# musevlt/muse-psfr

Measured on AMD Instinct MI355X. Metric: PSFs/sec (row x lambda) on 512^2 grid, 35 lambda, higher is better.
Workload: dtype f64 PSD->structure function, per-lambda OTF f32 -> split-fp16 MFMA (fp32 accumulate), f64 fit

## Files before the change

### muse_psfr_amd/csrc/dpp_groups.h

```cpp
#pragma once
#include "fft_lds.h"

namespace mpsfr {
namespace {

template <int L0>
__device__ __forceinline__ void cmac_group1(cx<double>& a0, double xr0, double xi0, const cx<double>& w) {
    asm("v_fmac_f64_dpp %0, %2, %4 row_newbcast:%6 row_mask:0xf bank_mask:0xf\n\t"
        "v_fmac_f64_dpp %1, %2, %5 row_newbcast:%6 row_mask:0xf bank_mask:0xf\n\t"
        "v_fmac_f64_dpp %0, -%3, %5 row_newbcast:%6 row_mask:0xf bank_mask:0xf\n\t"
        "v_fmac_f64_dpp %1, %3, %4 row_newbcast:%6 row_mask:0xf bank_mask:0xf"
        : "+v"(a0.x), "+v"(a0.y)
        : "v"(xr0), "v"(xi0), "v"(w.x), "v"(w.y), "n"(L0));
}

template <int L0>
__device__ __forceinline__ void rmac_group1(cx<double>& a0, double xr0, const cx<double>& w) {
    asm("v_fmac_f64_dpp %0, %2, %3 row_newbcast:%5 row_mask:0xf bank_mask:0xf\n\t"
        "v_fmac_f64_dpp %1, %2, %4 row_newbcast:%5 row_mask:0xf bank_mask:0xf"
        : "+v"(a0.x), "+v"(a0.y)
        : "v"(xr0), "v"(w.x), "v"(w.y), "n"(L0));
}

template <int L0, int L1>
__device__ __forceinline__ void cmac_group2(cx<double>& a0, cx<double>& a1, double xr0, double xi0, double xr1, double xi1, const cx<double>& w) {
    asm("v_fmac_f64_dpp %0, %4, %8 row_newbcast:%10 row_mask:0xf bank_mask:0xf\n\t"
        "v_fmac_f64_dpp %2, %6, %8 row_newbcast:%11 row_mask:0xf bank_mask:0xf\n\t"
        "v_fmac_f64_dpp %1, %4, %9 row_newbcast:%10 row_mask:0xf bank_mask:0xf\n\t"
        "v_fmac_f64_dpp %3, %6, %9 row_newbcast:%11 row_mask:0xf bank_mask:0xf\n\t"
        "v_fmac_f64_dpp %0, -%5, %9 row_newbcast:%10 row_mask:0xf bank_mask:0xf\n\t"
        "v_fmac_f64_dpp %2, -%7, %9 row_newbcast:%11 row_mask:0xf bank_mask:0xf\n\t"
        "v_fmac_f64_dpp %1, %5, %8 row_newbcast:%10 row_mask:0xf bank_mask:0xf\n\t"
        "v_fmac_f64_dpp %3, %7, %8 row_newbcast:%11 row_mask:0xf bank_mask:0xf"
        : "+v"(a0.x), "+v"(a0.y), "+v"(a1.x), "+v"(a1.y)
        : "v"(xr0), "v"(xi0), "v"(xr1), "v"(xi1), "v"(w.x), "v"(w.y), "n"(L0), "n"(L1));
}

template <int L0, int L1>
__device__ __forceinline__ void rmac_group2(cx<double>& a0, cx<double>& a1, double xr0, double xr1, const cx<double>& w) {
    asm("v_fmac_f64_dpp %0, %4, %6 row_newbcast:%8 row_mask:0xf bank_mask:0xf\n\t"
        "v_fmac_f64_dpp %2, %5, %6 row_newbcast:%9 row_mask:0xf bank_mask:0xf\n\t"
        "v_fmac_f64_dpp %1, %4, %7 row_newbcast:%8 row_mask:0xf bank_mask:0xf\n\t"
        "v_fmac_f64_dpp %3, %5, %7 row_newbcast:%9 row_mask:0xf bank_mask:0xf"
        : "+v"(a0.x), "+v"(a0.y), "+v"(a1.x), "+v"(a1.y)
        : "v"(xr0), "v"(xr1), "v"(w.x), "v"(w.y), "n"(L0), "n"(L1));
}

template <int L0, int L1, int L2, int L3>
__device__ __forceinline__ void cmac_group4(cx<double>& a0, cx<double>& a1, cx<double>& a2, cx<double>& a3, double xr0, double xi0, double xr1, double xi1, double xr2, double xi2, double xr3, double xi3, const cx<double>& w) {
    asm("v_fmac_f64_dpp %0, %8, %16 row_newbcast:%18 row_mask:0xf bank_mask:0xf\n\t"
        "v_fmac_f64_dpp %2, %10, %16 row_newbcast:%19 row_mask:0xf bank_mask:0xf\n\t"
        "v_fmac_f64_dpp %4, %12, %16 row_newbcast:%20 row_mask:0xf bank_mask:0xf\n\t"
        "v_fmac_f64_dpp %6, %14, %16 row_newbcast:%21 row_mask:0xf bank_mask:0xf\n\t"
        "v_fmac_f64_dpp %1, %8, %17 row_newbcast:%18 row_mask:0xf bank_mask:0xf\n\t"
        "v_fmac_f64_dpp %3, %10, %17 row_newbcast:%19 row_mask:0xf bank_mask:0xf\n\t"
        "v_fmac_f64_dpp %5, %12, %17 row_newbcast:%20 row_mask:0xf bank_mask:0xf\n\t"
        "v_fmac_f64_dpp %7, %14, %17 row_newbcast:%21 row_mask:0xf bank_mask:0xf\n\t"
        "v_fmac_f64_dpp %0, -%9, %17 row_newbcast:%18 row_mask:0xf bank_mask:0xf\n\t"
        "v_fmac_f64_dpp %2, -%11, %17 row_newbcast:%19 row_mask:0xf bank_mask:0xf\n\t"
        "v_fmac_f64_dpp %4, -%13, %17 row_newbcast:%20 row_mask:0xf bank_mask:0xf\n\t"
        "v_fmac_f64_dpp %6, -%15, %17 row_newbcast:%21 row_mask:0xf bank_mask:0xf\n\t"
        "v_fmac_f64_dpp %1, %9, %16 row_newbcast:%18 row_mask:0xf bank_mask:0xf\n\t"
        "v_fmac_f64_dpp %3, %11, %16 row_newbcast:%19 row_mask:0xf bank_mask:0xf\n\t"
        "v_fmac_f64_dpp %5, %13, %16 row_newbcast:%20 row_mask:0xf bank_mask:0xf\n\t"
        "v_fmac_f64_dpp %7, %15, %16 row_newbcast:%21 row_mask:0xf bank_mask:0xf"
        : "+v"(a0.x), "+v"(a0.y), "+v"(a1.x), "+v"(a1.y), "+v"(a2.x), "+v"(a2.y), "+v"(a3.x), "+v"(a3.y)
        : "v"(xr0), "v"(xi0), "v"(xr1), "v"(xi1), "v"(xr2), "v"(xi2), "v"(xr3), "v"(xi3), "v"(w.x), "v"(w.y), "n"(L0), "n"(L1), "n"(L2), "n"(L3));
}

template <int L0, int L1, int L2, int L3>
__device__ __forceinline__ void rmac_group4(cx<double>& a0, cx<double>& a1, cx<double>& a2, cx<double>& a3, double xr0, double xr1, double xr2, double xr3, const cx<double>& w) {
    asm("v_fmac_f64_dpp %0, %8, %12 row_newbcast:%14 row_mask:0xf bank_mask:0xf\n\t"
        "v_fmac_f64_dpp %2, %9, %12 row_newbcast:%15 row_mask:0xf bank_mask:0xf\n\t"
        "v_fmac_f64_dpp %4, %10, %12 row_newbcast:%16 row_mask:0xf bank_mask:0xf\n\t"
        "v_fmac_f64_dpp %6, %11, %12 row_newbcast:%17 row_mask:0xf bank_mask:0xf\n\t"
        "v_fmac_f64_dpp %1, %8, %13 row_newbcast:%14 row_mask:0xf bank_mask:0xf\n\t"
        "v_fmac_f64_dpp %3, %9, %13 row_newbcast:%15 row_mask:0xf bank_mask:0xf\n\t"
        "v_fmac_f64_dpp %5, %10, %13 row_newbcast:%16 row_mask:0xf bank_mask:0xf\n\t"
        "v_fmac_f64_dpp %7, %11, %13 row_newbcast:%17 row_mask:0xf bank_mask:0xf"
        : "+v"(a0.x), "+v"(a0.y), "+v"(a1.x), "+v"(a1.y), "+v"(a2.x), "+v"(a2.y), "+v"(a3.x), "+v"(a3.y)
        : "v"(xr0), "v"(xr1), "v"(xr2), "v"(xr3), "v"(w.x), "v"(w.y), "n"(L0), "n"(L1), "n"(L2), "n"(L3));
}

template <int L0, int L1, int L2, int L3, int L4>
__device__ __forceinline__ void cmac_group5(cx<double>& a0, cx<double>& a1, cx<double>& a2, cx<double>& a3, cx<double>& a4, double xr0, double xi0, double xr1, double xi1, double xr2, double xi2, double xr3, double xi3, double xr4, double xi4, const cx<double>& w) {
    asm("v_fmac_f64_dpp %0, %10, %20 row_newbcast:%22 row_mask:0xf bank_mask:0xf\n\t"
        "v_fmac_f64_dpp %2, %12, %20 row_newbcast:%23 row_mask:0xf bank_mask:0xf\n\t"
        "v_fmac_f64_dpp %4, %14, %20 row_newbcast:%24 row_mask:0xf bank_mask:0xf\n\t"
        "v_fmac_f64_dpp %6, %16, %20 row_newbcast:%25 row_mask:0xf bank_mask:0xf\n\t"
        "v_fmac_f64_dpp %8, %18, %20 row_newbcast:%26 row_mask:0xf bank_mask:0xf\n\t"
        "v_fmac_f64_dpp %1, %10, %21 row_newbcast:%22 row_mask:0xf bank_mask:0xf\n\t"
        "v_fmac_f64_dpp %3, %12, %21 row_newbcast:%23 row_mask:0xf bank_mask:0xf\n\t"
        "v_fmac_f64_dpp %5, %14, %21 row_newbcast:%24 row_mask:0xf bank_mask:0xf\n\t"
        "v_fmac_f64_dpp %7, %16, %21 row_newbcast:%25 row_mask:0xf bank_mask:0xf\n\t"
        "v_fmac_f64_dpp %9, %18, %21 row_newbcast:%26 row_mask:0xf bank_mask:0xf\n\t"
        "v_fmac_f64_dpp %0, -%11, %21 row_newbcast:%22 row_mask:0xf bank_mask:0xf\n\t"
        "v_fmac_f64_dpp %2, -%13, %21 row_newbcast:%23 row_mask:0xf bank_mask:0xf\n\t"
        "v_fmac_f64_dpp %4, -%15, %21 row_newbcast:%24 row_mask:0xf bank_mask:0xf\n\t"
        "v_fmac_f64_dpp %6, -%17, %21 row_newbcast:%25 row_mask:0xf bank_mask:0xf\n\t"
        "v_fmac_f64_dpp %8, -%19, %21 row_newbcast:%26 row_mask:0xf bank_mask:0xf\n\t"
        "v_fmac_f64_dpp %1, %11, %20 row_newbcast:%22 row_mask:0xf bank_mask:0xf\n\t"
        "v_fmac_f64_dpp %3, %13, %20 row_newbcast:%23 row_mask:0xf bank_mask:0xf\n\t"
        "v_fmac_f64_dpp %5, %15, %20 row_newbcast:%24 row_mask:0xf bank_mask:0xf\n\t"
        "v_fmac_f64_dpp %7, %17, %20 row_newbcast:%25 row_mask:0xf bank_mask:0xf\n\t"
        "v_fmac_f64_dpp %9, %19, %20 row_newbcast:%26 row_mask:0xf bank_mask:0xf"
        : "+v"(a0.x), "+v"(a0.y), "+v"(a1.x), "+v"(a1.y), "+v"(a2.x), "+v"(a2.y), "+v"(a3.x), "+v"(a3.y), "+v"(a4.x), "+v"(a4.y)
        : "v"(xr0), "v"(xi0), "v"(xr1), "v"(xi1), "v"(xr2), "v"(xi2), "v"(xr3), "v"(xi3), "v"(xr4), "v"(xi4), "v"(w.x), "v"(w.y), "n"(L0), "n"(L1), "n"(L2), "n"(L3), "n"(L4));
}

template <int L0, int L1, int L2, int L3, int L4>
__device__ __forceinline__ void rmac_group5(cx<double>& a0, cx<double>& a1, cx<double>& a2, cx<double>& a3, cx<double>& a4, double xr0, double xr1, double xr2, double xr3, double xr4, const cx<double>& w) {
    asm("v_fmac_f64_dpp %0, %10, %15 row_newbcast:%17 row_mask:0xf bank_mask:0xf\n\t"
        "v_fmac_f64_dpp %2, %11, %15 row_newbcast:%18 row_mask:0xf bank_mask:0xf\n\t"
        "v_fmac_f64_dpp %4, %12, %15 row_newbcast:%19 row_mask:0xf bank_mask:0xf\n\t"
        "v_fmac_f64_dpp %6, %13, %15 row_newbcast:%20 row_mask:0xf bank_mask:0xf\n\t"
        "v_fmac_f64_dpp %8, %14, %15 row_newbcast:%21 row_mask:0xf bank_mask:0xf\n\t"
        "v_fmac_f64_dpp %1, %10, %16 row_newbcast:%17 row_mask:0xf bank_mask:0xf\n\t"
        "v_fmac_f64_dpp %3, %11, %16 row_newbcast:%18 row_mask:0xf bank_mask:0xf\n\t"
        "v_fmac_f64_dpp %5, %12, %16 row_newbcast:%19 row_mask:0xf bank_mask:0xf\n\t"
        "v_fmac_f64_dpp %7, %13, %16 row_newbcast:%20 row_mask:0xf bank_mask:0xf\n\t"
        "v_fmac_f64_dpp %9, %14, %16 row_newbcast:%21 row_mask:0xf bank_mask:0xf"
        : "+v"(a0.x), "+v"(a0.y), "+v"(a1.x), "+v"(a1.y), "+v"(a2.x), "+v"(a2.y), "+v"(a3.x), "+v"(a3.y), "+v"(a4.x), "+v"(a4.y)
        : "v"(xr0), "v"(xr1), "v"(xr2), "v"(xr3), "v"(xr4), "v"(w.x), "v"(w.y), "n"(L0), "n"(L1), "n"(L2), "n"(L3), "n"(L4));
}

}
}
```

### muse_psfr_amd/csrc/kernels.h

```cpp
#pragma once
#include <hip/hip_runtime.h>
#include <stdint.h>

namespace mpsfr {

constexpr int NS = 40;
constexpr int NSH = NS / 2 + 1;
constexpr int KS = 41;
constexpr int NAO = 80;
constexpr int NFIT = 16;
constexpr int NFIT_ELL = 24;
constexpr int NFIT_PSF = 16;
constexpr int METRIC_MAX = 16;
constexpr int METRIC_HEAD = 8;
constexpr int KHAT = 33 * 64;
constexpr int MAXLGS = 4;

struct TaskPar {
    double r0m53;
    double inv_l0sq;
    double cn2_0;
    double cn2_1;
    int geom;
    int basis;
};

struct LamPar {
    double c;
    int npixc;
    int pad;
};

struct AoGeom {
    double h[2];
    double wind[2][2];
    int nlgs[2];
    double poslgs[2][2][MAXLGS];
    int ndir;
    double dir[2][25];
};

constexpr int MAXLAYER = 8;
struct AoLayers {
    int n;
    int ntab;
    double h[MAXLAYER];
    double wind[2][MAXLAYER];
};
inline int ao_ntab(int nlayer) { return nlayer < 2 ? 2 : nlayer; }
struct LayerMix {
    const double* w = nullptr;
    int ntab = 2;
};

constexpr int kMfLists = 64;
constexpr int kMfSchedInts = kMfLists + 1;

enum KernelId {
    K_AO_TABLES = 0,
    K_TEL_OTF,
    K_PSD_ROWFFT,
    K_COLFFT_DPHI,
    K_GTABLE,
    K_MOFFAT_KERNELS,
    K_OTF_ROWFFT,
    K_COLPASS,
    K_CONV,
    K_FIT,
    K_STAMP_SUM,
    K_VKEEP,
    K_OTF_MFMA,
    K_MF_PREP,
    K_PATCH,
    K_DPHI_SERIES,
    K_COUNT
};

void launch_ao_tables(hipStream_t s, const AoGeom& g, const uint8_t* d_mask_rec,
                      const uint8_t* d_mask_res, double* d_tab);
void launch_ao_tables_profile(hipStream_t s, const AoGeom& g, const AoLayers& ly, const uint8_t* d_mask_rec,
                              const uint8_t* d_mask_res, double* d_tab);
void launch_tel_otf(hipStream_t s, int N, const uint64_t* d_rows, int words, double pupsum,
                    void* d_tel, bool f64out);
int psd_rowfft_groups(int N);
void launch_psd_rowfft(hipStream_t s, int N, int ntd, int ndir, const TaskPar* d_tp,
                       const double* d_aotab, double cfit, void* d_C, const void* d_tw64,
                       double* d_dcpart, bool f64, const LayerMix& mix = LayerMix());
void launch_colfft_dphi(hipStream_t s, int N, int ntd, const void* d_C, const double* d_dcpart,
                        double scale2, void* d_D0t, bool f64out, const void* d_tw64,
                        int* d_zero = nullptr);
void launch_dmin(hipStream_t s, int N, int ntd, const void* d_D0t, float* d_dline, float* d_dblk,
                 bool f64 = false);
void launch_psd_image(hipStream_t s, int N, int ndir, const TaskPar& p, const double* d_aotab, double cfit,
                      double unit, double* d_psd, const LayerMix& mix = LayerMix());
void launch_dphi_from_psd(hipStream_t s, int N, int ndir, const double* d_psd, void* d_Cm, double scale,
                          void* d_D0t, bool f64out, const void* d_tw64);
bool p2p_supported(int M);
void launch_p2p_otf(hipStream_t s, int M, int P, int nz, const double* d_pup, const double* d_phase,
                    const double* d_lbda_m, double scale, void* d_T1, void* d_Q, double* d_otft, const void* d_twm);
void launch_p2p_psf(hipStream_t s, int M, int N, int nz, const double* d_D0t, const double* d_otft, size_t otf_stride,
                    const double* d_cl, void* d_G, double* d_psf, const void* d_twm);
size_t series_twiddle_bytes(int N);
void launch_series_twiddles(hipStream_t s, int N, const void* d_tw64, void* d_twk);
int series_terms(bool f64);
double series_eps0();
inline double series_eps_max() { return 1.0 / 49.0; }
void launch_series_coef(hipStream_t s, int N, const double* d_planes, void* d_coef, bool f64);
struct SeriesQueue {
    int* queue = nullptr;
    const int* perm = nullptr;
    const float* tlmax = nullptr;
    float c2max = 0.f, thr_elem = -3.0e38f, thr_mass = -3.0e38f;
};
struct PatchExtras {
    const void* blob_src = nullptr;
    void* blob_dst = nullptr;
    size_t blob_bytes = 0;
    const TaskPar* tp_host = nullptr;
    unsigned long long* flag = nullptr;
    unsigned long long seq = 0;
    int* queue_zero = nullptr;
    int khat_n = 0;
    const double* khat_gam = nullptr;
    const double* khat_alp = nullptr;
    void* khat_out = nullptr;
    bool khat_f64 = false;
};
void launch_patch(hipStream_t s, int N, int ntd, int ndir, const TaskPar* d_tp, const double* d_aotab,
                  double cfit, const void* d_twk, double* d_P, void* d_T, double* d_sp, bool f64,
                  const PatchExtras& x = PatchExtras(), const LayerMix& mix = LayerMix());
void launch_dphi_series(hipStream_t s, int N, int ntd, int ndir, const TaskPar* d_tp, const void* d_T,
                        const double* d_sp, const void* d_coef, const void* d_twk, double scale2,
                        void* d_D0t, float* d_dlin, bool f64out, int* d_zero, int ncu,
                        const unsigned* d_support = nullptr, const SeriesQueue& qx = SeriesQueue());
void launch_series_support(hipStream_t s, int N, const void* d_tel, bool f64, unsigned* d_support);
void launch_dmin16(hipStream_t s, int N, int ntd, const float* d_dlin, float* d_dline, float* d_dblk);
void launch_tel_linemax(hipStream_t s, int N, const void* d_tel, float* d_tlmax, bool f64 = false);
void launch_vkeep(hipStream_t s, int N, int ntask, int ndir, int nl, const LamPar* d_lp,
                  const float* d_dline, const float* d_dblk, const float* d_tlmax, float thr_sum,
                  int* d_vkeep, int fixed, float* d_dminb);
void launch_task_order(hipStream_t s, int ntask, int nl, const int* d_vkeep, int* d_order);
size_t mf_etab_bytes(int N, int nl);
size_t mf_gtab_bytes(int N, int nl);
size_t mf_tl2_bytes(int N);
size_t mf_tlb_bytes(int N);
size_t mf_dminb_bytes(int N, int ntask);
int mf_block_count(int N);
void launch_mf_tables(hipStream_t s, int N, int nl, const LamPar* d_lp, const void* d_tw64,
                      void* d_E, void* d_G);
void launch_mf_tel(hipStream_t s, int N, const void* d_tel, float* d_tl2, float* d_tlb);
void launch_peak_floor(hipStream_t s, int N, int ntask, int ndir, const void* d_D0t, const float* d_tl2, float c2min,
                       float tier_half, float floor_nominal, float* d_thrf);
void launch_otf_mfma(hipStream_t s, int N, int ntask, int ndir, int nl, const void* d_D0t,
                     const float* d_tl2, const LamPar* d_lp, const void* d_E, const void* d_G,
                     const int* d_vkeep, const float* d_dminb, const float* d_tlb, float thr,
                     void* d_pre, const int* d_order = nullptr, void* d_clk = nullptr, const float* d_thrf = nullptr);
size_t mf2_own_bytes(int N, int ntask, int nl);
size_t mf2_uni_bytes(int N, int ntask, int nl);
size_t mf2_sched_bytes(int N, int ntask, int nl, int permax);
size_t mf2_part_bytes(int N, int ntask, int nl);
void mf2_groups(int nl, int permax, int* per, int* ngr);
void launch_mf_prep(hipStream_t s, int N, int ntask, int nl, int permax, const LamPar* d_lp,
                    const float* d_dminb, const float* d_tlb, float thr, float thr_floor, float thr_mid,
                    float tier_half, const void* d_D0t, const float* d_tl2, void* d_own,
                    void* d_uni, void* d_sched, const float* d_dlin = nullptr);
void launch_otf_mfma2(hipStream_t s, int N, int ntask, int nl, int permax, int ncu, const void* d_D0t,
                      const float* d_tl2, const LamPar* d_lp, const void* d_E, const void* d_G,
                      const void* d_own, const void* d_uni, void* d_sched, void* d_part, void* d_pre,
                      void* d_clk = nullptr, hipEvent_t ev_start = nullptr, hipEvent_t ev_stop = nullptr,
                      bool finish = true);
struct MfFinishArgs {
    const int* gsw = nullptr;
    const void* part = nullptr;
    int per = 1, ngr = 1, nsw = 1;
};
MfFinishArgs mf2_finish_args(int N, int ntask, int nl, int permax, void* d_sched, const void* d_part);
void launch_mf_finish(hipStream_t s, int N, int ntask, int nl, int permax, void* d_sched, const void* d_part, void* d_pre);
void launch_gtable(hipStream_t s, int N, int nl, const LamPar* d_lp, const void* d_tw64,
                   int* d_samp_p, void* d_samp_a, void* d_G, bool f64);
void launch_moffat_kernels(hipStream_t s, int nker, const double* d_gamma, const double* d_alpha,
                           void* d_out, bool f64);
void launch_otf_rowfft(hipStream_t s, int N, int ntask, int ndir, int nl, const void* d_D0t,
                       const void* d_tel, const LamPar* d_lp, const int* d_samp_p,
                       const void* d_samp_a, const void* d_xtab, void* d_Tq, const void* d_tw64,
                       bool f64, bool fast_exp, const int* d_vkeep);
bool otf_uses_r16(int N, bool f64, int nl, int ndir);
size_t xtab_bytes(int nl);
void launch_xtab(hipStream_t s, int N, int nl, const int* d_samp_p, const void* d_samp_a,
                 const void* d_tw64, void* d_xtab);
void launch_colpass(hipStream_t s, int N, int ntask, int nl, const void* d_Tq, const void* d_G,
                    void* d_pre, bool f64, const int* d_vkeep);
void launch_conv(hipStream_t s, int ntask, int nl, const void* d_pre, const void* d_ktt,
                 const void* d_kmuse, double* d_fin, bool f64, int tdiv = 1);
void launch_khat(hipStream_t s, int nker, const double* d_gamma, const double* d_alpha,
                 void* d_khat, bool f64 = false);
void launch_conv_fft(hipStream_t s, int ntask, int nl, const void* d_pre, const void* d_khat_tt,
                     const void* d_khat_muse, void* d_fin, bool fin_f32, bool f64 = false,
                     const MfFinishArgs& finish = MfFinishArgs(), int tdiv = 1);
void launch_fit(hipStream_t s, int nstamp, const void* d_stamps, bool stamps_f32, double* d_fit,
                bool f64, int sum_ntask = 0, int sum_nl = 0, double* d_sum = nullptr, int sum_accumulate = 0);
void launch_stamp_sum(hipStream_t s, int ntask, int nl, const void* d_fin, bool fin_f32, double* d_sum,
                      int accumulate);
void launch_fit_ell(hipStream_t s, int nstamp, const double* d_stamps, double* d_fit, bool f64);
void launch_fit_obs(hipStream_t s, int nstamp, const double* d_stamps, const double* d_var, int flags, double* d_fit,
                    bool f64);
void launch_fit_psf(hipStream_t s, int nstamp, const double* d_stamps, const double* d_var, int npsf,
                    const double* d_psf, const int32_t* d_index, const double* d_shift, int flags, double* d_fit,
                    bool f64);
void launch_stamp_metrics(hipStream_t s, int nstamp, const double* d_stamps, const double* d_centers, int nrad,
                          const double* radii, int nbox, const double* boxes, int nfrac, const double* fractions,
                          double* d_out);
constexpr int MAX_BANDS = 16;
int band_stride(int nband);
void launch_band_reduce(hipStream_t s, int ntb, int nl, int nband, const void* d_fin, bool fin_f32,
                        const double* d_w, double* d_out);
void launch_param_copy(hipStream_t s, void* d_dst, const void* h_src_pinned, size_t bytes,
                       unsigned long long* h_flag_pinned = nullptr, unsigned long long seq = 0);

}
```

### muse_psfr_amd/csrc/mpsfr_api.cpp

```cpp
#include "../../include/mpsfr.h"

#include <hip/hip_runtime.h>

#include <algorithm>
#include <chrono>
#include <cmath>
#include <cstdarg>
#include <cstdio>
#include <cstring>
#include <string>
#include <thread>
#include <vector>

#include "coeff_l0_table.h"
#include "kernels.h"

using namespace mpsfr;

namespace {

thread_local std::string g_err;

constexpr float kMfFloorLog2 = -29.01f;

// ... 784 lines not shown
static_assert(MAX_BANDS == MPSFR_MAX_BANDS, "K_BAND_REDUCE keeps MPSFR_MAX_BANDS accumulators");

int mpsfr_reconstruct_band(mpsfr_ctx* c, int ntask, const double* seeing, const double* gl, const double* l0,
                           const uint8_t* three_lgs, const double h[2], double wind_speed, int npsflin, int npos,
                           const double* pos_arcsec, int nl, const double* lbda_nm, int nband, const double* weights,
                           const uint8_t* mask_rec, const uint8_t* mask_res, double* band_out, double* band_sum_out,
                           double* band_fit_out, int on_device) {
    if (!c) return fail(MPSFR_E_INVALID, "ctx is NULL");
    if (nband < 1 || nband > MPSFR_MAX_BANDS) return fail(MPSFR_E_INVALID, "nband=%d out of range 1..%d", nband, MPSFR_MAX_BANDS);
    if (nl < 1 || nl > 4096) return fail(MPSFR_E_INVALID, "nl=%d out of range", nl);
    if (!weights) return fail(MPSFR_E_INVALID, "weights is NULL");
    std::vector<double> w((size_t)nband * nl);
    for (int b = 0; b < nband; ++b) {
        const double* r = weights + (size_t)b * nl;
        double sum = 0.0;
        for (int l = 0; l < nl; ++l) {
            if (!std::isfinite(r[l]) || r[l] < 0.0) return fail(MPSFR_E_INVALID, "band %d: weight %d must be finite and >= 0", b, l);
            sum += r[l];
        }
        if (!(sum > 0.0) || !std::isfinite(sum)) return fail(MPSFR_E_INVALID, "band %d: the weights sum to %g", b, sum);
        for (int l = 0; l < nl; ++l) w[(size_t)b * nl + l] = r[l] / sum;
    }
    StageIO io;
    io.nband = nband;
    io.bw = w.data();
    if (npos < 0 || npos > 25) return fail(MPSFR_E_INVALID, "npos=%d out of range 0..25", npos);
    if (npos > 0) {
        if (npsflin != 0) return fail(MPSFR_E_INVALID, "a field call (npos >= 1) takes npsflin = 0");
        if (!pos_arcsec) return fail(MPSFR_E_INVALID, "pos_arcsec is NULL");
        for (int k = 0; k < 2 * npos; ++k)
            if (!std::isfinite(pos_arcsec[k]) || std::fabs(pos_arcsec[k]) > 60.0)
                return fail(MPSFR_E_INVALID, "position %d: need finite |x|, |y| <= 60 arcsec", k / 2);
        io.npos = npos;
        io.pos = pos_arcsec;
        npsflin = 1;
    } else if (npsflin < 1 || npsflin > 5) {
        return fail(MPSFR_E_INVALID, "npsflin=%d out of range 1..5", npsflin);
    }
    return guarded_call(c, ntask, seeing, gl, l0, three_lgs, h, wind_speed, npsflin, nl, lbda_nm, mask_rec, mask_res,
                        band_out, band_sum_out, band_fit_out, on_device, io);
}

static_assert(MAXLAYER == MPSFR_MAX_LAYERS, "AoLayers holds MPSFR_MAX_LAYERS layers");

static int profile_layers(int ntask, int nlayer, const double* h, const double* wind_speed, const double* wind_dir,
                          const double* cn2, AoLayers& ly, std::vector<double>& w) {
    if (nlayer < 1 || nlayer > MPSFR_MAX_LAYERS) return fail(MPSFR_E_INVALID, "nlayer=%d out of range 1..%d", nlayer, MPSFR_MAX_LAYERS);
    if (!h || !wind_speed || !wind_dir || !cn2) return fail(MPSFR_E_INVALID, "NULL profile array");
    memset(&ly, 0, sizeof ly);
    ly.n = nlayer;
    ly.ntab = ao_ntab(nlayer);
    for (int l = 0; l < nlayer; ++l) {
        if (!std::isfinite(h[l]) || !std::isfinite(wind_speed[l]) || !std::isfinite(wind_dir[l]))
            return fail(MPSFR_E_INVALID, "layer %d: non-finite altitude or wind", l);
        if (h[l] < 0.0 || h[l] > 50000.0) return fail(MPSFR_E_INVALID, "layer %d: h=%g outside [0, 50000] m", l, h[l]);
        if (wind_speed[l] < 0.0 || wind_speed[l] > 100.0)
            return fail(MPSFR_E_INVALID, "layer %d: wind speed %g outside [0, 100] m/s", l, wind_speed[l]);
        ly.h[l] = h[l];
        ly.wind[0][l] = wind_speed[l] * std::cos(wind_dir[l]);
        ly.wind[1][l] = wind_speed[l] * std::sin(wind_dir[l]);
    }
    for (int t = 0; t < ntask; ++t) {
        double sum = 0.0;
        for (int l = 0; l < nlayer; ++l) {
            const double w = cn2[(size_t)t * nlayer + l];
            if (!std::isfinite(w) || w < 0.0) return fail(MPSFR_E_INVALID, "row %d: weight %d must be finite and >= 0", t, l);
            sum += w;
        }
        if (!(sum > 0.0) || !std::isfinite(sum)) return fail(MPSFR_E_INVALID, "row %d: the weights sum to %g", t, sum);
    }
    int keep[MAXLAYER], nk = 0;
    for (int l = 0; l < nlayer; ++l) {
        bool used = false;
        for (int t = 0; t < ntask && !used; ++t) used = cn2[(size_t)t * nlayer + l] != 0.0;
        if (used) keep[nk++] = l;
    }
    for (int k = 0; k < nk; ++k) {
        ly.h[k] = ly.h[keep[k]];
        ly.wind[0][k] = ly.wind[0][keep[k]];
        ly.wind[1][k] = ly.wind[1][keep[k]];
    }
    for (int k = nk; k < MAXLAYER; ++k) ly.h[k] = ly.wind[0][k] = ly.wind[1][k] = 0.0;
    ly.n = nk;
    ly.ntab = ao_ntab(nk);
    w.resize((size_t)ntask * nk);
    for (int t = 0; t < ntask; ++t)
        for (int k = 0; k < nk; ++k) w[(size_t)t * nk + k] = cn2[(size_t)t * nlayer + keep[k]];
    return MPSFR_OK;
}

int mpsfr_reconstruct_profile(mpsfr_ctx* c, int ntask, const double* seeing, const double* gl,
                              const double* l0, const uint8_t* three_lgs,
                              int nlayer, const double* h, const double* wind_speed, const double* wind_dir,
                              const double* cn2, int npsflin, int npos, const double* pos_arcsec,
                              int nl, const double* lbda_nm, const uint8_t* mask_rec, const uint8_t* mask_res,
                              double* psf_out, double* psf_sum_out, double* fit_out, int on_device) {
    if (!c) return fail(MPSFR_E_INVALID, "ctx is NULL");
    if (ntask < 1) return fail(MPSFR_E_INVALID, "ntask < 1");
    AoLayers ly;
    std::vector<double> w;
    int rc = profile_layers(ntask, nlayer, h, wind_speed, wind_dir, cn2, ly, w);
    if (rc) return rc;
    StageIO io;
    io.layers = &ly;
    io.cn2 = w.data();
    if (npos < 0 || npos > 25) return fail(MPSFR_E_INVALID, "npos=%d out of range 0..25", npos);
    if (npos > 0) {
        if (npsflin != 0) return fail(MPSFR_E_INVALID, "a field call (npos >= 1) takes npsflin = 0");
        if (!pos_arcsec) return fail(MPSFR_E_INVALID, "pos_arcsec is NULL");
        for (int k = 0; k < 2 * npos; ++k)
            if (!std::isfinite(pos_arcsec[k]) || std::fabs(pos_arcsec[k]) > 60.0)
                return fail(MPSFR_E_INVALID, "position %d: need finite |x|, |y| <= 60 arcsec", k / 2);
        io.npos = npos;
        io.pos = pos_arcsec;
        npsflin = 1;
    } else if (npsflin < 1 || npsflin > 5) {
        return fail(MPSFR_E_INVALID, "npsflin=%d out of range 1..5", npsflin);
    }
    const double h2[2] = {0.0, 0.0};
    return guarded_call(c, ntask, seeing, gl, l0, three_lgs, h2, 0.0, npsflin, nl, lbda_nm, mask_rec, mask_res,
                        psf_out, psf_sum_out, fit_out, on_device, io);
}

int mpsfr_simul_psd_profile(mpsfr_ctx* c, double seeing, double l0, int three_lgs,
                            int nlayer, const double* h, const double* wind_speed, const double* wind_dir,
                            const double* cn2, int npsflin, int npos, const double* pos_arcsec,
                            const uint8_t* mask_rec, const uint8_t* mask_res, double* psd_out) {
    if (!c || !psd_out) return fail(MPSFR_E_INVALID, "NULL argument");
    AoLayers ly;
    std::vector<double> w;
    int rc = profile_layers(1, nlayer, h, wind_speed, wind_dir, cn2, ly, w);
    if (rc) return rc;
    StageIO io;
    io.layers = &ly;
    io.cn2 = w.data();
    io.psd_out = psd_out;
    if (npos < 0 || npos > 25) return fail(MPSFR_E_INVALID, "npos=%d out of range 0..25", npos);
    if (npos > 0) {
        if (npsflin != 0) return fail(MPSFR_E_INVALID, "positions (npos >= 1) take npsflin = 0");
        if (!pos_arcsec) return fail(MPSFR_E_INVALID, "pos_arcsec is NULL");
        for (int k = 0; k < 2 * npos; ++k)
            if (!std::isfinite(pos_arcsec[k]) || std::fabs(pos_arcsec[k]) > 60.0)
                return fail(MPSFR_E_INVALID, "position %d: need finite |x|, |y| <= 60 arcsec", k / 2);
        io.npos = npos;
        io.pos = pos_arcsec;
        npsflin = 1;
    } else if (npsflin < 1 || npsflin > 5) {
        return fail(MPSFR_E_INVALID, "npsflin=%d out of range 1..5", npsflin);
    }
    const uint8_t t3 = three_lgs ? 1 : 0;
    const double lb = 700.0;
    const double h2[2] = {0.0, 0.0};
    const double gl = 0.5;
    return guarded_call(c, 1, &seeing, &gl, &l0, &t3, h2, 0.0, npsflin, 1, &lb, mask_rec, mask_res,
                        nullptr, nullptr, nullptr, 0, io);
}

static int reconstruct_impl(mpsfr_ctx* c, int ntask, const double* seeing, const double* gl,
                            const double* l0, const uint8_t* three_lgs, const double h[2],
                            double wind_speed, int npsflin, int nl, const double* lbda_nm,
                            const uint8_t* mask_rec, const uint8_t* mask_res, double* psf_out,
                            double* psf_sum_out, double* fit_out, int on_device, const StageIO& io) {
    const auto t_enter = std::chrono::steady_clock::now();
    const bool staged = io.psd_out || io.psd_in || io.pre_in || io.stop_pre;
    if (staged && on_device != 0) return fail(MPSFR_E_INVALID, "stage-level calls take host buffers");
    if (ntask < 1 || !seeing || !gl || !l0 || !h || !lbda_nm)
        return fail(MPSFR_E_INVALID, "ntask < 1 or NULL input array");
    if (nl < 1 || nl > 4096) return fail(MPSFR_E_INVALID, "nl=%d out of range", nl);
    const bool field = io.npos > 0;
    if (field && ((staged && !io.psd_out) || !io.pos)) return fail(MPSFR_E_INVALID, "field call without positions");
    if (!field && (npsflin < 1 || npsflin > 5)) return fail(MPSFR_E_INVALID, "npsflin=%d out of range 1..5", npsflin);
    if ((mask_rec == nullptr) != (mask_res == nullptr))
        return fail(MPSFR_E_INVALID, "mask_rec and mask_res must both be given or both be NULL");
    const int N = c->N, H1 = N / 2 + 1, ndir = field ? io.npos : npsflin * npsflin;
    const int gpp = field ? ndir : 1, ndb = field ? 1 : ndir;
    const bool band = io.nband > 0;
    if (band && (staged || !io.bw || io.nband > MAX_BANDS)) return fail(MPSFR_E_INVALID, "bad band request");
    const int nout = band ? io.nband : nl;
    HIPCHK(hipSetDevice(c->device));
    int rc;

    std::vector<LamPar> lp(nl);
    std::vector<double> gam, alp;
    for (int l = 0; l < nl; ++l) {
        if (!(lbda_nm[l] > 0.0)) return fail(MPSFR_E_INVALID, "lbda[%d] must be > 0", l);
        const double k = 2.0 * M_PI / lbda_nm[l];
        lp[l].c = -0.5 * k * k;
        lp[l].npixc = npix_crop(lbda_nm[l], c->dimpsf, c->pixscale);
        lp[l].pad = 0;
        if (!io.pre_in && !io.psd_out && (lp[l].npixc > N || lp[l].npixc < NS))
            return fail(MPSFR_E_GRID,
                        "lbda=%.3f nm needs a %d-pixel crop, outside [%d, dim=%d] "
                        "(psfrec.py:663-683)", lbda_nm[l], lp[l].npixc, NS, N);
    }
    const AoLayers* ly = io.layers;
    const int ntab = ly ? ly->ntab : 2;
    std::vector<double> wts;
    int low = 0;
    if (ly) {
        if (!io.cn2) return fail(MPSFR_E_INVALID, "profile call without weights");
        wts.assign((size_t)ntask * ntab, 0.0);
        for (int l = 1; l < ly->n; ++l)
            if (ly->h[l] < ly->h[low]) low = l;
        for (int t = 0; t < ntask; ++t) {
            const double* r = io.cn2 + (size_t)t * ly->n;
            double sum = 0.0;
            for (int l = 0; l < ly->n; ++l) sum += r[l];
            for (int l = 0; l < ly->n; ++l) wts[(size_t)t * ntab + l] = r[l] / sum;
        }
    }
    std::vector<TaskPar> tp(ntask);
    gam.resize((size_t)ntask + nl);
    alp.resize((size_t)ntask + nl);
    for (int t = 0; t < ntask; ++t) {
        if (!(seeing[t] > 0.0) || !(l0[t] > 0.0) || !(gl[t] >= 0.0) || !(gl[t] <= 1.0))
            return fail(MPSFR_E_INVALID, "task %d: need seeing > 0, L0 > 0, 0 <= GL <= 1", t);
        const double r0 = 0.976 * 0.5 / seeing[t] / 4.85;
        double c0 = gl[t], c1 = 1.0 - gl[t];
        const double cs = c0 + c1;
        c0 /= cs;
        c1 /= cs;
        tp[t].r0m53 = std::pow(r0, -5.0 / 3.0);
        tp[t].inv_l0sq = (1.0 / l0[t]) * (1.0 / l0[t]);
        tp[t].cn2_0 = c0;
        tp[t].cn2_1 = c1;
        if (io.layers) {
            tp[t].cn2_0 = wts[(size_t)t * ntab + low];
            tp[t].cn2_1 = 1.0 - tp[t].cn2_0;
        }
        tp[t].geom = (three_lgs && three_lgs[t]) ? 1 : 0;
        tp[t].basis = 0;
        gam[t] = tiptilt_alpha(seeing[t], gl[t], l0[t], c->pixscale);
        alp[t] = 2.0;
    }
    for (int l = 0; l < nl; ++l) muse_kernel_params(lbda_nm[l], c->pixscale, &gam[ntask + l], &alp[ntask + l]);
    bool series = c->stage_a == 2 || (c->stage_a == 1 && (N >= 512 || (N >= 256 && ndir >= 2)));
    if (io.psd_in) series = false;
    for (int t = 0; t < ntask; ++t) series = series && tp[t].inv_l0sq <= series_eps_max();

    AoGeom g;
    memset(&g, 0, sizeof g);
    g.h[0] = h[0];
    g.h[1] = h[1];
    const double arg_v[2] = {0.628163, -0.326497};
    for (int l = 0; l < 2; ++l) {
        g.wind[0][l] = wind_speed * std::cos(arg_v[l]);
        g.wind[1][l] = wind_speed * std::sin(arg_v[l]);
    }
    const double pos4[4][2] = {{1, 1}, {-1, -1}, {-1, 1}, {1, -1}};
    g.nlgs[0] = 4;
    g.nlgs[1] = 3;
    for (int ge = 0; ge < 2; ++ge)
        for (int q = 0; q < g.nlgs[ge]; ++q) {
            g.poslgs[ge][0][q] = pos4[q][0] * 63.0 / 60;
            g.poslgs[ge][1][q] = pos4[q][1] * 63.0 / 60;
        }
    g.ndir = ndir;
    for (int d = 0; d < ndir; ++d) {
        if (field) {
            g.dir[0][d] = io.pos[2 * d] / 60;
            g.dir[1][d] = io.pos[2 * d + 1] / 60;
        } else {
            g.dir[0][d] = (double)(d / npsflin - npsflin / 2) * 60 / 2 / 60;
            g.dir[1][d] = (double)(d % npsflin - npsflin / 2) * 60 / 2 / 60;
        }
    }

    mpsfr_ctx::Ticket* tk = nullptr;
    if (on_device == 2) {
        tk = &c->ticket[c->ticket_next % mpsfr_ctx::NTICKET];
        if ((rc = complete_ticket(c, *tk))) return rc;
        tk->u_psf = psf_out;
        tk->u_sum = psf_sum_out;
        tk->u_fit = fit_out;
        tk->n_psf = psf_out ? (size_t)ntask * gpp * nout * NS * NS : 0;
        tk->n_sum = psf_sum_out ? (size_t)gpp * nout * NS * NS : 0;
        tk->n_fit = fit_out ? (size_t)ntask * gpp * nout * NFIT : 0;
        const size_t hb = (tk->n_psf + tk->n_sum + tk->n_fit) * sizeof(double);
        if (hb > tk->host_cap) {
            if (tk->host) HIPCHK(hipHostFree(tk->host));
            tk->host = nullptr;
            tk->host_cap = 0;
            HIPCHK(hipHostMalloc(&tk->host, hb + hb / 8, hipHostMallocDefault));
            tk->host_cap = hb + hb / 8;
        }
        if (tk->n_psf && (rc = ensure(c, tk->dpsf, tk->n_psf * sizeof(double)))) return rc;
        if (tk->n_sum && (rc = ensure(c, tk->dsum, tk->n_sum * sizeof(double)))) return rc;
        if (tk->n_fit && (rc = ensure(c, tk->dfit, tk->n_fit * sizeof(double)))) return rc;
        if (!tk->done) HIPCHK(hipEventCreateWithFlags(&tk->done, hipEventDisableTiming));
        psf_out = tk->n_psf ? (double*)tk->dpsf.p : nullptr;
        psf_sum_out = tk->n_sum ? (double*)tk->dsum.p : nullptr;
        fit_out = tk->n_fit ? (double*)tk->dfit.p : nullptr;
        on_device = 1;
    }

    const int NLmax = c->nlanes == 0 ? 2 : c->nlanes;
    int TC = c->chunk_tasks;
    if (TC <= 0) {
        const int spt = gpp * nl + (band ? gpp * nout : 0);
        int big = 65536 / spt;
        const int soft = (4096 + spt - 1) / spt < 8 ? 8 : (4096 + spt - 1) / spt;
        if (big > 512) big = 512;
        if (big < soft) big = soft;
        const double per_task = series ? (double)ndir * H1 * (N * (double)rsize(c) + NAO * 16.0)
                                       : (double)ndir * (N / 2 + NAO / 2) * H1 * 16.0;
        const int cap = (int)(4.0 * 1024 * 1024 * 1024 / per_task);
        if (big > cap) big = cap < 1 ? 1 : cap;
        int nch = (ntask + big - 1) / big;
        if (nch > 1) nch = (nch + NLmax - 1) / NLmax * NLmax;
        if (nch == 1 && NLmax > 1 && (long)ntask * spt >= 8192 && !(c->pipeline_calls && on_device != 0))
            nch = NLmax;
        TC = (ntask + nch - 1) / nch;
    }
    if (staged && !io.pre_in) TC = ntask;
    if (TC > ntask) TC = ntask;
    const int nchunks = (ntask + TC - 1) / TC;
    const int NL = NLmax < nchunks ? NLmax : nchunks;
    const bool dev_out = on_device != 0;
    const bool join = c->stream_exported || tk != nullptr || !dev_out || NL > 1 || !c->pipeline_calls;
    const bool lean = !join;
    if (!(c->pipeline_calls && dev_out)) c->lane_rr = 0;
    const int L0 = (int)(c->lane_rr % (unsigned)NLmax);
    c->lane_rr += (unsigned)nchunks;
    auto lane_of = [&](int j) -> mpsfr_ctx::Lane& { return c->lane[(L0 + j) % NLmax]; };
    for (int j = 0; j < NL; ++j) {
        mpsfr_ctx::Lane& ln = lane_of(j);
        if (!ln.stream) {
            const int li = (int)(&ln - c->lane);
            if (c->cu_partition && NLmax > 1) {
                const int lo = c->ncu * li / NLmax, hi = c->ncu * (li + 1) / NLmax;
                uint32_t mask[16] = {0};
                for (int b = lo; b < hi && b < 512; ++b) mask[b >> 5] |= 1u << (b & 31);
                HIPCHK(hipExtStreamCreateWithCUMask(&ln.stream, (uint32_t)((c->ncu + 31) / 32), mask));
                ln.ncu = hi - lo;
            } else {
                HIPCHK(hipStreamCreateWithFlags(&ln.stream, hipStreamNonBlocking));
                ln.ncu = 0;
            }
        }
        if (!ln.done) HIPCHK(hipEventCreateWithFlags(&ln.done, hipEventDisableTiming));
    }
    hipStream_t s0 = lane_of(0).stream;
    const int stagger = c->cold_stagger;
    bool cold_first = false;
    if (stagger && NLmax > 1) {
        cold_first = true;
        for (int k = 0; k < mpsfr_ctx::MAX_LANES; ++k)
            if (c->lane[k].busy && (c->lane[k].marked ? hipEventQuery(c->lane[k].done_ev) : hipStreamQuery(c->lane[k].stream)) != hipSuccess)
                cold_first = false;
        if (!c->stagger_ev) HIPCHK(hipEventCreateWithFlags(&c->stagger_ev, hipEventDisableTiming));
    }

    if ((rc = ensure(c, c->aotab, (size_t)2 * ndir * (ntab + 1) * NAO * NAO * sizeof(double)))) return rc;
    const size_t ko = sizeof(AoGeom) + 1 + (ly ? sizeof(AoLayers) : 0);
    std::vector<unsigned char> key(ko + 1 + (mask_rec ? 2 * NAO * NAO : 0));
    memcpy(key.data(), &g, sizeof(AoGeom));
    key[sizeof(AoGeom)] = ly ? 1 : 0;
    if (ly) {
        AoLayers lk;
        memset(&lk, 0, sizeof lk);
        lk.n = ly->n;
        lk.ntab = ly->ntab;
        for (int l = 0; l < ly->n; ++l) {
            lk.h[l] = ly->h[l];
            lk.wind[0][l] = ly->wind[0][l];
            lk.wind[1][l] = ly->wind[1][l];
        }
        memcpy(key.data() + sizeof(AoGeom) + 1, &lk, sizeof lk);
    }
    key[ko] = mask_rec ? 1 : 0;
    if (mask_rec) {
        memcpy(key.data() + ko + 1, mask_rec, NAO * NAO);
        memcpy(key.data() + ko + 1 + NAO * NAO, mask_res, NAO * NAO);
    }
    const bool need_ao = !io.pre_in && !io.psd_in;
    const bool ao_cached = !need_ao || (key == c->cache_geom && c->cache_ao_ptr == c->aotab.p);
    const bool send_masks = mask_rec && !ao_cached;

    auto al16 = [](size_t x) { return (x + 15) & ~(size_t)15; };
    const size_t o_lp = 0;
    const size_t o_tp = al16(o_lp + nl * sizeof(LamPar));
    const size_t o_gam = al16(o_tp + ntask * sizeof(TaskPar));
    const size_t o_alp = al16(o_gam + gam.size() * sizeof(double));
    const size_t o_mr = al16(o_alp + alp.size() * sizeof(double));
    const size_t o_ms = al16(o_mr + (send_masks ? NAO * NAO : 0));
    const bool want_perm = c->stage_a_queue != 0 && series;
    const size_t o_perm = al16(o_ms + (send_masks ? NAO * NAO : 0));
    const size_t o_w = al16(o_perm + (want_perm ? (size_t)ntask * ndir * sizeof(int) : 0));
    const int bstride = band ? band_stride(nout) : 0;
    const size_t o_bw = al16(o_w + wts.size() * sizeof(double));
    const size_t blob = al16(o_bw + (size_t)nl * bstride * sizeof(double));
    mpsfr_ctx::Slot& sl = c->slot[c->stage_next++ % mpsfr_ctx::NSTAGE];
    double t_blocked = 0.0;
    if (sl.staged_pending) {
        const auto tb = std::chrono::steady_clock::now();
        if (sl.staged_mode == 2) {
            volatile unsigned long long* flag = c->seq_host + (&sl - c->slot);
            const auto t_lim = tb + std::chrono::seconds(5);
            for (long spins = 0; *flag < sl.seq; ++spins) {
                if (spins < 4096) {
#if defined(__x86_64__) || defined(__i386__)
                    __builtin_ia32_pause();
#elif defined(__aarch64__)
                    asm volatile("yield" ::: "memory");
#endif
                    continue;
                }
                std::this_thread::yield();
                if ((spins & 255) == 0 && std::chrono::steady_clock::now() > t_lim) {
                    if (sl.last_lane >= 0 && c->lane[sl.last_lane].stream)
                        HIPCHK(hipStreamSynchronize(c->lane[sl.last_lane].stream));
                    else
                        HIPCHK(hipDeviceSynchronize());
                    break;
                }
            }
        } else {
            HIPCHK(hipEventSynchronize(sl.staged_ev));
        }
        t_blocked = std::chrono::duration<double>(std::chrono::steady_clock::now() - tb).count();
        sl.staged_pending = false;
    }
    if (blob > sl.host_cap) {
        if (sl.host) HIPCHK(hipHostFree(sl.host));
        sl.host = nullptr;
        sl.host_cap = 0;
        HIPCHK(hipHostMalloc(&sl.host, blob * 2, hipHostMallocDefault));
        sl.host_cap = blob * 2;
    }
    if (!sl.staged) HIPCHK(hipEventCreateWithFlags(&sl.staged, hipEventDisableTiming));
    if (!sl.call_done) HIPCHK(hipEventCreateWithFlags(&sl.call_done, hipEventDisableTiming));
    const bool use_fft_conv = c->fft_conv;
    const size_t ksz = use_fft_conv ? (size_t)KHAT * 2 * rsize(c) : (size_t)KS * KS * rsize(c);
    if ((rc = ensure(c, sl.params, blob))) return rc;
    if ((rc = ensure(c, sl.ktt, (size_t)ntask * ksz))) return rc;
    char* hb = (char*)sl.host;
    memcpy(hb + o_lp, lp.data(), nl * sizeof(LamPar));
    memcpy(hb + o_tp, tp.data(), ntask * sizeof(TaskPar));
    memcpy(hb + o_gam, gam.data(), gam.size() * sizeof(double));
    memcpy(hb + o_alp, alp.data(), alp.size() * sizeof(double));
    if (ly) memcpy(hb + o_w, wts.data(), wts.size() * sizeof(double));
    if (band) {
        double* bw = reinterpret_cast<double*>(hb + o_bw);
        for (int l = 0; l < nl; ++l)
            for (int b = 0; b < bstride; ++b) bw[(size_t)l * bstride + b] = b < nout ? io.bw[(size_t)b * nl + l] : 0.0;
    }
    if (want_perm) {
        int* pm = reinterpret_cast<int*>(hb + o_perm);
        std::vector<int> idx;
        for (int t0 = 0; t0 < ntask; t0 += TC) {
            const int tc = (ntask - t0) < TC ? (ntask - t0) : TC;
            idx.resize(tc);
            for (int k = 0; k < tc; ++k) idx[k] = k;
            auto key = [&](int k) { return tp[t0 + k].r0m53 * tp[t0 + k].cn2_1 * std::pow(tp[t0 + k].inv_l0sq, -5.0 / 6.0); };
            std::stable_sort(idx.begin(), idx.end(), [&](int a, int b) { return key(a) > key(b); });
            for (int k = 0; k < tc; ++k)
                for (int d = 0; d < ndir; ++d) pm[(size_t)(t0 + k) * ndir + d] = idx[k] * ndir + d;
        }
    }
    if (send_masks) {
        memcpy(hb + o_mr, mask_rec, NAO * NAO);
        memcpy(hb + o_ms, mask_res, NAO * NAO);
    }
    const void* outs[3] = {dev_out ? (const void*)psf_out : nullptr,
                           dev_out ? (const void*)psf_sum_out : nullptr,
                           dev_out ? (const void*)fit_out : nullptr};
    if (c->wait_next && hipEventQuery(c->wait_next) == hipSuccess) c->wait_next = nullptr;
    const bool slot_done = sl.call_pending && sl.has_event && hipEventQuery(sl.call_done) == hipSuccess;
    for (int j = 0; j < NL; ++j) {
        hipStream_t ls = lane_of(j).stream;
        if (sl.call_pending && !slot_done && sl.last_lane != (int)(&lane_of(j) - c->lane)) {
            if (sl.has_event) HIPCHK(hipStreamWaitEvent(ls, sl.call_done, 0));
            else if (sl.last_lane >= 0) HIPCHK(hipStreamWaitEvent(ls, lane_end(c, c->lane[sl.last_lane]), 0));
        }
        if (c->wait_next) HIPCHK(hipStreamWaitEvent(ls, c->wait_next, 0));
        if (c->lsum_busy && NL > 1) HIPCHK(hipStreamWaitEvent(ls, c->lsum_done, 0));
        for (int k = 0; k < mpsfr_ctx::MAX_LANES; ++k) {
            mpsfr_ctx::Lane& o = c->lane[k];
            if (&o == &lane_of(j) || !o.busy) continue;
            bool same = false;
            for (int hsl = 0; hsl < mpsfr_ctx::Lane::NHIST; ++hsl)
                for (int a = 0; a < 3; ++a)
                    for (int b = 0; b < 3; ++b) same = same || (outs[a] && outs[a] == o.outs[hsl][b]);
            if (same) HIPCHK(hipStreamWaitEvent(ls, lane_end(c, o), 0));
        }
    }
    c->wait_next = nullptr;
    sl.call_pending = false;
    if ((rc = ensure(c, c->samp_p, (size_t)nl * NS * sizeof(int)))) return rc;
    if ((rc = ensure(c, c->samp_a, (size_t)nl * NS * rsize(c)))) return rc;
    if ((rc = ensure(c, c->G, (size_t)nl * ((H1 + 7) / 8 * 8) * NS * 2 * rsize(c)))) return rc;
    if ((rc = ensure(c, c->kmuse, (size_t)nl * ksz))) return rc;
    const bool mf = !c->f64 && c->otf_mfma;
    const bool mf2 = mf && ndb == 1 && c->mf_kernel == 2;
    const bool r16 = !mf && otf_uses_r16(N, c->f64, nl, ndb);
    const bool fuse_finish = mf2 && c->finish_fusion && c->fft_conv && !io.stop_pre && !io.pre_in;
    if (r16 && (rc = ensure(c, c->xtab, xtab_bytes(nl)))) return rc;
    if (mf) {
        if ((rc = ensure(c, c->etab, mf_etab_bytes(N, nl)))) return rc;
        if ((rc = ensure(c, c->gtab, mf_gtab_bytes(N, nl)))) return rc;
    }
    const bool need_lam = !io.psd_out;
    const std::vector<double> lb_key(lbda_nm, lbda_nm + nl);
    const bool lam_cached = !need_lam || (lb_key == c->cache_lbda && c->cache_lbda_mode == (use_fft_conv ? 1 : 0) &&
                            c->cache_G_ptr == c->G.p && c->cache_kmuse_ptr == c->kmuse.p &&
                            (!r16 || (c->cache_xtab_valid && c->cache_xtab_ptr == c->xtab.p)) &&
                            (!mf || (c->cache_mf_valid && c->cache_etab_ptr == c->etab.p &&
                                     c->cache_gtab_ptr == c->gtab.p)));
    const bool zero = lean && c->param_copy_kernel && c->seq_host != nullptr;
    const bool fuse_head = c->head_fusion && series && !staged;
    const bool fuse_copy = fuse_head && c->copy_fusion && c->param_copy_kernel && NL == 1 && lam_cached && ao_cached &&
                           !ly;
    const bool fuse_khat = fuse_head && c->fft_conv;
    sl.seq = ++c->seq_next;
    if (zero) {
        if (!fuse_copy) launch_param_copy(s0, sl.params.p, hb, blob, c->seq_host + (&sl - c->slot), sl.seq);
        sl.staged_mode = 2;
    } else {
        if (fuse_copy) ;
        else if (c->param_copy_kernel) launch_param_copy(s0, sl.params.p, hb, blob, nullptr, 0);
        else HIPCHK(hipMemcpyAsync(sl.params.p, hb, blob, hipMemcpyHostToDevice, s0));
        if (lean) {
            sl.staged_ev = sl.call_done;
            sl.staged_mode = 1;
        } else {
            if (!fuse_copy) HIPCHK(hipEventRecord(sl.staged, s0));
            sl.staged_ev = sl.staged;
            sl.staged_mode = 0;
        }
    }
    sl.staged_pending = true;
    const char* db = (const char*)sl.params.p;
    const LamPar* d_lp = (const LamPar*)(db + o_lp);
    const TaskPar* d_tp = (const TaskPar*)(db + o_tp);
    const double* d_gam = (const double*)(db + o_gam);
    const double* d_alp = (const double*)(db + o_alp);
    const double* d_w = ly ? (const double*)(db + o_w) : nullptr;
    const double* d_bw = band ? (const double*)(db + o_bw) : nullptr;
    auto mix_of = [&](int t0) {
        LayerMix m;
        m.w = ly ? d_w + (size_t)t0 * ntab : nullptr;
        m.ntab = ntab;
        return m;
    };
    const uint8_t* d_mrec = send_masks ? (const uint8_t*)(db + o_mr) : nullptr;
    const uint8_t* d_mres = send_masks ? (const uint8_t*)(db + o_ms) : nullptr;

    if (!ao_cached || !lam_cached) {
        for (int k = 0; k < mpsfr_ctx::MAX_LANES; ++k)
            if (c->lane[k].busy && c->lane[k].stream != s0)
                HIPCHK(hipStreamWaitEvent(s0, lane_end(c, c->lane[k]), 0));
        if (!ao_cached) {
            ProfScope ps(c, K_AO_TABLES, s0);
            if (ly) launch_ao_tables_profile(s0, g, *ly, d_mrec, d_mres, (double*)c->aotab.p);
            else launch_ao_tables(s0, g, d_mrec, d_mres, (double*)c->aotab.p);
            c->cache_geom.swap(key);
            c->last_ntab = ntab;
            c->cache_ao_ptr = c->aotab.p;
        }
        if (!lam_cached) {
            {
                ProfScope ps(c, K_GTABLE, s0);
                launch_gtable(s0, N, nl, d_lp, c->tw64.p, (int*)c->samp_p.p, c->samp_a.p, c->G.p,
                              c->f64);
                if (r16)
                    launch_xtab(s0, N, nl, (const int*)c->samp_p.p, c->samp_a.p, c->tw64.p, c->xtab.p);
                if (mf) launch_mf_tables(s0, N, nl, d_lp, c->tw64.p, c->etab.p, c->gtab.p);
            }
            ProfScope ps(c, K_MOFFAT_KERNELS, s0);
            if (use_fft_conv) launch_khat(s0, nl, d_gam + ntask, d_alp + ntask, c->kmuse.p, c->f64);
            else launch_moffat_kernels(s0, nl, d_gam + ntask, d_alp + ntask, c->kmuse.p, c->f64);
            c->cache_lbda = lb_key;
            c->cache_lbda_mode = use_fft_conv ? 1 : 0;
            c->cache_G_ptr = c->G.p;
            c->cache_kmuse_ptr = c->kmuse.p;
            c->cache_xtab_ptr = c->xtab.p;
            c->cache_xtab_valid = r16;
            c->cache_etab_ptr = c->etab.p;
            c->cache_gtab_ptr = c->gtab.p;
            c->cache_mf_valid = mf;
        }
        if (!c->cache_ready) HIPCHK(hipEventCreateWithFlags(&c->cache_ready, hipEventDisableTiming));
        HIPCHK(hipEventRecord(c->cache_ready, s0));
        c->cache_ready_valid = true;
    } else if (c->cache_ready_valid) {
        if (hipEventQuery(c->cache_ready) == hipSuccess) c->cache_ready_valid = false;
        else HIPCHK(hipStreamWaitEvent(s0, c->cache_ready, 0));
    }
    {
        ProfScope ps(c, K_MOFFAT_KERNELS, s0);
        if (fuse_khat) ;
        else if (use_fft_conv) launch_khat(s0, ntask, d_gam, d_alp, sl.ktt.p, c->f64);
        else launch_moffat_kernels(s0, ntask, d_gam, d_alp, sl.ktt.p, c->f64);
    }

    const size_t per_stamp = (size_t)NS * NS;
    const int TB = TC * gpp;
    const double eps_prune = c->f64 ? c->prune_eps_f64 : c->prune_eps;
    const bool prune = eps_prune > 0.0;
    const float thr_sum = prune ? (float)((mf ? 0.5 : 1.0) * eps_prune / (2.0 * N * ndb)) : 0.f;
    float thr_blk = (prune && mf)
        ? (float)std::log2(0.5 * eps_prune / (2.0 * ndb * 16 * 32 * mf_block_count(N))) : 0.f;
    const float thr_eps = thr_blk;
    float thr_floor = -1.0e30f;
    const bool tiers = prune && mf && c->tier_eps > 0.0;
    const bool floor_per_task = tiers && c->mf_floor && !mf2 && std::isfinite(c->tier_eps);
    if (tiers && c->mf_floor) {
        thr_floor = (float)c->mf_floor_log2;
        if (!mf2 && !floor_per_task && thr_blk < thr_floor) thr_blk = thr_floor;
    }
    float c2min = 0.f;
    for (int l = 0; l < nl; ++l) c2min = std::fmin(c2min, (float)(lp[l].c * 1.44269504088896340736));
    const float thr_mid = (tiers && c->mf_floor) ? (float)c->mf_mid_log2 : -1.0e30f;
    float tier_half = std::isfinite(c->tier_eps) ? (float)(0.5 * c->tier_eps) : 0.f;
    const bool line_skip = c->stage_a_queue == 2 && mf2 && series && prune && !staged;
    float c2max = -3.0e38f;
    for (int l = 0; l < nl; ++l) c2max = std::fmax(c2max, (float)(lp[l].c * 1.44269504088896340736));
    float line_mass_log2 = -3.0e38f;
    if (line_skip && tiers && c->mf_floor && tier_half > 0.f) {
        line_mass_log2 = (float)std::log2(c->tier_eps / 8.0 / (double)H1);
        tier_half *= 0.75f;
    }
    for (int j = 0; j < NL; ++j) {
        mpsfr_ctx::Lane& ln = lane_of(j);
        if ((rc = ensure(c, ln.pre, (size_t)TB * nl * per_stamp * (c->f64 ? 8 : 4)))) return rc;
        if ((rc = ensure(c, ln.fin, (size_t)TB * nl * per_stamp * sizeof(double)))) return rc;
        if (band && !(dev_out && psf_out) && (rc = ensure(c, ln.band, (size_t)TB * nout * per_stamp * sizeof(double))))
            return rc;
        if (io.pre_in) continue;
        if (series) {
            if ((rc = ensure(c, ln.pP, (size_t)TC * ndir * NAO * NAO * sizeof(double)))) return rc;
            if ((rc = ensure(c, ln.pT, (size_t)TC * ndir * H1 * NAO * 2 * sizeof(double)))) return rc;
            if ((rc = ensure(c, ln.psp, (size_t)TC * ndir * sizeof(double)))) return rc;
            if (c->stage_a_queue && (rc = ensure(c, ln.squeue, 64))) return rc;
            if (prune && (rc = ensure(c, ln.dlin, (size_t)TC * ndir * H1 * (N / 32) * sizeof(float)))) return rc;
        } else {
            if ((rc = ensure(c, ln.C, (size_t)TC * ndir * (N / 2 + NAO / 2) * H1 * 2 * sizeof(double)))) return rc;
            if ((rc = ensure(c, ln.s00, (size_t)TC * ndir * psd_rowfft_groups(N) * sizeof(double)))) return rc;
        }
        {
            const size_t cap_before = ln.D0t.cap;
            if ((rc = ensure(c, ln.D0t, ((size_t)TC * ndir * H1 + 16) * N * rsize(c)))) return rc;
            if (ln.D0t.cap != cap_before) {
                HIPCHK(hipMemset(ln.D0t.p, 0, ln.D0t.cap));
                ln.d0t_stale = 0;
            }
        }
        if (!mf && (rc = ensure(c, ln.Tq, (size_t)TB * nl * H1 * NSH * 2 * rsize(c)))) return rc;
        if (mf2) {
            if ((rc = ensure(c, ln.mown, mf2_own_bytes(N, TB, nl)))) return rc;
            if ((rc = ensure(c, ln.muni, mf2_uni_bytes(N, TB, nl)))) return rc;
            if ((rc = ensure(c, ln.msched, mf2_sched_bytes(N, TB, nl, c->mf_permax)))) return rc;
            if ((rc = ensure(c, ln.mpart, mf2_part_bytes(N, TB, nl)))) return rc;
        }
        if (prune) {
            if ((rc = ensure(c, ln.dmin, (size_t)TC * ndir * H1 * sizeof(float)))) return rc;
            if ((rc = ensure(c, ln.dblk, (size_t)ndir * mf_dminb_bytes(N, TC)))) return rc;
            if (mf && (rc = ensure(c, ln.dminb, mf_dminb_bytes(N, TB)))) return rc;
            if (mf && (rc = ensure(c, ln.order, (size_t)TB * sizeof(int)))) return rc;
            if (mf && (rc = ensure(c, ln.thrf, (size_t)TB * sizeof(float)))) return rc;
            if ((rc = ensure(c, ln.vkeep, (size_t)TB * ((nl + 1) / 2) * sizeof(int)))) return rc;
        }
    }
    const int nsum = gpp * nout;
    if (NL > 1 && (rc = ensure(c, c->lsum, (size_t)NL * nsum * per_stamp * sizeof(double)))) return rc;
    if ((rc = ensure(c, c->sum, (size_t)nsum * per_stamp * sizeof(double)))) return rc;
    double* d_fin_all = nullptr;
    double* d_fit_all = nullptr;
    if (dev_out && psf_out && !band) d_fin_all = psf_out;
    if (dev_out && fit_out) {
        d_fit_all = fit_out;
    } else {
        if ((rc = ensure(c, c->fit, (size_t)ntask * gpp * nout * NFIT * sizeof(double)))) return rc;
        d_fit_all = (double*)c->fit.p;
    }
    const double cfit = fit_constant();
    const double scale2 = dphi_scale2();
    double* d_sum = (dev_out && psf_sum_out) ? psf_sum_out : (double*)c->sum.p;

    if (NL > 1) {
        if (!c->tables_ready) HIPCHK(hipEventCreateWithFlags(&c->tables_ready, hipEventDisableTiming));
        HIPCHK(hipEventRecord(c->tables_ready, s0));
        for (int j = 1; j < NL; ++j) HIPCHK(hipStreamWaitEvent(lane_of(j).stream, c->tables_ready, 0));
    }
    if (io.psd_out) {
        const size_t n = (size_t)ndir * N * N;
        DevBuf img;
        if ((rc = ensure(c, img, n * sizeof(double)))) return rc;
        launch_psd_image(s0, N, ndir, tp[0], (const double*)c->aotab.p, cfit, dphi_scale2() * 128.0, (double*)img.p,
                         mix_of(0));
        const hipError_t e1 = hipMemcpyAsync(io.psd_out, img.p, n * sizeof(double), hipMemcpyDeviceToHost, s0);
        const hipError_t e2 = hipStreamSynchronize(s0);
        release(img);
        if (e1 != hipSuccess || e2 != hipSuccess) return fail(MPSFR_E_HIP, "copying the PSD image failed");
        return MPSFR_OK;
    }
    bool lanes_shared = NL > 1;
    if (!lanes_shared && NLmax > 1 && c->pipeline_calls && (c->reserve_mf < 0 || c->reserve_a < 0))
        for (int k = 0; k < mpsfr_ctx::MAX_LANES; ++k) {
            const mpsfr_ctx::Lane& o = c->lane[k];
            if (&o == &lane_of(0) || !o.busy || !o.stream) continue;
            if ((o.marked ? hipEventQuery(o.done_ev) : hipStreamQuery(o.stream)) != hipSuccess) lanes_shared = true;
        }
    int nchunk_lane[mpsfr_ctx::MAX_LANES] = {0, 0, 0, 0};
    int ci = 0;
    for (int t0 = 0; t0 < ntask; t0 += TC, ++ci) {
        const int tc = (ntask - t0) < TC ? (ntask - t0) : TC;
        const int ntd = tc * ndir;
        const int tb = tc * gpp;
        const int j = ci % NL;
        mpsfr_ctx::Lane& ln = lane_of(j);
        hipStream_t ls = ln.stream;
        const int lane_index = (int)(&ln - c->lane);
        if (c->stagger_armed && lane_index != c->stagger_lane) {
            HIPCHK(hipStreamWaitEvent(ls, c->stagger_ev, 0));
            c->stagger_armed = false;
        }
        if (!io.pre_in) {
            const bool skip_form = series && c->support_skip;
            if (ln.d0t_stale == 2 || (ln.d0t_stale == 1 && skip_form)) {
                HIPCHK(hipMemsetAsync(ln.D0t.p, 0, ln.D0t.cap, ls));
                ln.d0t_stale = 0;
                ++c->d0t_clears;
            }
            if (io.psd_in) ln.d0t_stale = 2;
            else if (!skip_form && ln.d0t_stale < 1) ln.d0t_stale = 1;
        }
        if (io.pre_in) {
            const size_t n = (size_t)tc * nl * per_stamp;
            if (c->f64) {
                HIPCHK(hipMemcpyAsync(ln.pre.p, io.pre_in + (size_t)t0 * nl * per_stamp, n * sizeof(double),
                                      hipMemcpyHostToDevice, ls));
                HIPCHK(hipStreamSynchronize(ls));
            } else {
                std::vector<float> tmp(n);
                for (size_t i = 0; i < n; ++i) tmp[i] = (float)io.pre_in[(size_t)t0 * nl * per_stamp + i];
                HIPCHK(hipMemcpyAsync(ln.pre.p, tmp.data(), n * sizeof(float), hipMemcpyHostToDevice, ls));
                HIPCHK(hipStreamSynchronize(ls));
            }
        } else if (io.psd_in) {
            const size_t n = (size_t)ndir * N * N;
            DevBuf img, cm;
            if ((rc = ensure(c, img, n * sizeof(double)))) return rc;
            if ((rc = ensure(c, cm, (size_t)ndir * N * H1 * 2 * sizeof(double)))) { release(img); return rc; }
            hipError_t e1 = hipMemcpyAsync(img.p, io.psd_in, n * sizeof(double), hipMemcpyHostToDevice, ls);
            launch_dphi_from_psd(ls, N, ndir, (const double*)img.p, cm.p, 2.0 / 256.0, ln.D0t.p, c->f64, c->tw64.p);
            if (mf2 && e1 == hipSuccess) e1 = hipMemsetAsync(ln.msched.p, 0, kMfSchedInts * sizeof(int), ls);
            const hipError_t e2 = hipStreamSynchronize(ls);
            release(img);
            release(cm);
            if (e1 != hipSuccess || e2 != hipSuccess) return fail(MPSFR_E_HIP, "the structure function of the PSD failed");
        } else if (series) {
            {
                ProfScope ps(c, K_PATCH, ls);
                PatchExtras px;
                if (fuse_copy && t0 == 0) {
                    px.blob_src = hb;
                    px.blob_dst = sl.params.p;
                    px.blob_bytes = blob;
                    px.tp_host = (const TaskPar*)(hb + o_tp);
                    px.flag = zero ? c->seq_host + (&sl - c->slot) : nullptr;
                    px.seq = sl.seq;
                }
                if (c->stage_a_queue) px.queue_zero = (int*)ln.squeue.p;
                if (fuse_khat) {
                    px.khat_n = tc;
                    px.khat_gam = d_gam + t0;
                    px.khat_alp = d_alp + t0;
                    px.khat_out = (char*)sl.ktt.p + (size_t)t0 * ksz;
                    px.khat_f64 = c->f64;
                }
                launch_patch(ls, N, ntd, ndir, d_tp + t0, (const double*)c->aotab.p, cfit, c->stwk.p,
                             (double*)ln.pP.p, ln.pT.p, (double*)ln.psp.p, c->f64, px, mix_of(t0));
                if (fuse_copy && t0 == 0 && !zero && !lean) HIPCHK(hipEventRecord(sl.staged, ls));
            }
            ProfScope ps(c, K_DPHI_SERIES, ls);
            SeriesQueue sq;
            if (c->stage_a_queue) {
                sq.queue = (int*)ln.squeue.p;
                sq.perm = reinterpret_cast<const int*>(db + o_perm) + (size_t)t0 * ndir;
                if (line_skip) {
                    sq.tlmax = (const float*)c->tlmax.p;
                    sq.c2max = c2max;
                    sq.thr_elem = thr_eps;
                    sq.thr_mass = line_mass_log2;
                }
            }
            launch_dphi_series(ls, N, ntd, ndir, d_tp + t0, ln.pT.p, (const double*)ln.psp.p, c->scoef.p,
                               c->stwk.p, scale2, ln.D0t.p, prune ? (float*)ln.dlin.p : nullptr, c->f64,
                               mf2 ? (int*)ln.msched.p : nullptr, persist_grid(c, ln, c->reserve_a, lanes_shared),
                               c->support_skip ? (const unsigned*)c->ssup.p : nullptr, sq);
        } else {
            {
                ProfScope ps(c, K_PSD_ROWFFT, ls);
                launch_psd_rowfft(ls, N, ntd, ndir, d_tp + t0, (const double*)c->aotab.p, cfit, ln.C.p,
                                  c->tw64.p, (double*)ln.s00.p, c->f64, mix_of(t0));
            }
            ProfScope ps(c, K_COLFFT_DPHI, ls);
            launch_colfft_dphi(ls, N, ntd, ln.C.p, (const double*)ln.s00.p, scale2, ln.D0t.p,
                               c->f64, c->tw64.p, mf2 ? (int*)ln.msched.p : nullptr);
        }
        auto stagger_here = [&](int which) -> int {
            if (cold_first && stagger == which) {
                if (hipEventRecord(c->stagger_ev, ls) != hipSuccess) return -1;
                c->stagger_armed = true;
                c->stagger_lane = lane_index;
                cold_first = false;
            }
            return 0;
        };
        if (stagger_here(1)) return fail(MPSFR_E_HIP, "hipEventRecord failed");
        if (io.pre_in) {
        } else if (mf2) {
            ProfScope ps(c, K_MF_PREP, ls);
            const bool from_lines = prune && series && !io.psd_in;
            if (prune && !from_lines) launch_dmin(ls, N, ntd, ln.D0t.p, (float*)ln.dmin.p, (float*)ln.dblk.p);
            launch_mf_prep(ls, N, tb, nl, c->mf_permax, d_lp, (prune && !from_lines) ? (const float*)ln.dblk.p : nullptr,
                           (const float*)c->tlb.p, thr_eps, thr_floor, thr_mid, tier_half, ln.D0t.p, (const float*)c->tl2.p,
                           ln.mown.p, ln.muni.p, ln.msched.p, from_lines ? (const float*)ln.dlin.p : nullptr);
        } else if (prune) {
            ProfScope ps(c, mf ? K_MF_PREP : K_VKEEP, ls);
            if (series) launch_dmin16(ls, N, ntd, (const float*)ln.dlin.p, (float*)ln.dmin.p, (float*)ln.dblk.p);
            else launch_dmin(ls, N, ntd, ln.D0t.p, (float*)ln.dmin.p, (float*)ln.dblk.p, c->f64);
            launch_vkeep(ls, N, tb, ndb, nl, d_lp, (const float*)ln.dmin.p, (const float*)ln.dblk.p,
                         (const float*)c->tlmax.p, thr_sum, (int*)ln.vkeep.p, c->prune_fixed,
                         mf ? (float*)ln.dminb.p : nullptr);
            if (mf) launch_task_order(ls, tb, nl, (const int*)ln.vkeep.p, (int*)ln.order.p);
        }
        const int* d_vkeep = prune ? (const int*)ln.vkeep.p : nullptr;
        if (stagger_here(2)) return fail(MPSFR_E_HIP, "hipEventRecord failed");
        if (io.pre_in) {
        } else if (mf2) {
            ProfScope ps(c, K_OTF_MFMA, ls, false);
            launch_otf_mfma2(ls, N, tb, nl, c->mf_permax, persist_grid(c, ln, c->reserve_mf, lanes_shared), ln.D0t.p, (const float*)c->tl2.p, d_lp, c->etab.p,
                             c->gtab.p, ln.mown.p, ln.muni.p, ln.msched.p, ln.mpart.p, ln.pre.p,
                             c->mf_clock ? c->mfclk.p : nullptr, ps.a, ps.b, !fuse_finish);
        } else if (mf) {
            ProfScope ps(c, K_OTF_MFMA, ls);
            if (floor_per_task)
                launch_peak_floor(ls, N, tb, ndb, ln.D0t.p, (const float*)c->tl2.p, c2min, tier_half, thr_floor,
                                  (float*)ln.thrf.p);
            launch_otf_mfma(ls, N, tb, ndb, nl, ln.D0t.p, (const float*)c->tl2.p, d_lp, c->etab.p,
                            c->gtab.p, d_vkeep, prune ? (const float*)ln.dminb.p : nullptr,
                            (const float*)c->tlb.p, thr_blk, ln.pre.p,
                            prune ? (const int*)ln.order.p : nullptr, c->mf_clock ? c->mfclk.p : nullptr,
                            floor_per_task ? (const float*)ln.thrf.p : nullptr);
        } else {
            {
                ProfScope ps(c, K_OTF_ROWFFT, ls);
                launch_otf_rowfft(ls, N, tb, ndb, nl, ln.D0t.p, c->tel.p, d_lp,
                                  (const int*)c->samp_p.p, c->samp_a.p, c->xtab.p, ln.Tq.p, c->tw64.p,
                                  c->f64, c->fast_exp, d_vkeep);
            }
            ProfScope ps(c, K_COLPASS, ls);
            launch_colpass(ls, N, tb, nl, ln.Tq.p, c->G.p, ln.pre.p, c->f64, d_vkeep);
        }
        if (io.stop_pre) {
            const size_t n = (size_t)tc * nl * per_stamp;
            if (c->f64) {
                HIPCHK(hipMemcpyAsync(psf_out + (size_t)t0 * nl * per_stamp, ln.pre.p, n * sizeof(double),
                                      hipMemcpyDeviceToHost, ls));
                HIPCHK(hipStreamSynchronize(ls));
            } else {
                std::vector<float> tmp(n);
                HIPCHK(hipMemcpyAsync(tmp.data(), ln.pre.p, n * sizeof(float), hipMemcpyDeviceToHost, ls));
                HIPCHK(hipStreamSynchronize(ls));
                for (size_t i = 0; i < n; ++i) psf_out[(size_t)t0 * nl * per_stamp + i] = (double)tmp[i];
            }
            HIPCHK(hipGetLastError());
            ++nchunk_lane[j];
            c->last_chunk_tasks = tc;
            c->last_lane = (L0 + j) % NLmax;
            continue;
        }
        const bool fin_f32 = band ? (use_fft_conv && !c->f64)
                                  : (use_fft_conv && !c->f64 && !d_fin_all && !(psf_out && !dev_out));
        void* d_fin = d_fin_all ? (void*)(d_fin_all + (size_t)t0 * nsum * per_stamp) : ln.fin.p;
        {
            ProfScope ps(c, K_CONV, ls);
            const size_t koff = (size_t)t0 * ksz;
            if (use_fft_conv)
                launch_conv_fft(ls, tb, nl, ln.pre.p, (const char*)sl.ktt.p + koff,
                                c->kmuse.p, d_fin, fin_f32, c->f64,
                                fuse_finish ? mf2_finish_args(N, tb, nl, c->mf_permax, ln.msched.p, ln.mpart.p) : MfFinishArgs(),
                                gpp);
            else
                launch_conv(ls, tb, nl, ln.pre.p, (const char*)sl.ktt.p + koff,
                            c->kmuse.p, (double*)d_fin, c->f64, gpp);
        }
        void* d_res = d_fin;
        bool res_f32 = fin_f32;
        if (band) {
            ProfScope ps(c, K_STAMP_SUM, ls);
            double* d_band = (dev_out && psf_out) ? psf_out + (size_t)t0 * nsum * per_stamp : (double*)ln.band.p;
            launch_band_reduce(ls, tb, nl, nout, d_fin, fin_f32, d_bw, d_band);
            d_res = d_band;
            res_f32 = false;
        }
        double* lsum = NL > 1 ? (double*)c->lsum.p + (size_t)j * nsum * per_stamp : d_sum;
        if (fit_out) {
            ProfScope ps(c, K_FIT, ls);
            launch_fit(ls, tb * nout, d_res, res_f32, d_fit_all + (size_t)t0 * nsum * NFIT, c->f64,
                       psf_sum_out ? tc : 0, nsum, psf_sum_out ? lsum : nullptr, nchunk_lane[j] > 0 ? 1 : 0);
        } else if (psf_sum_out) {
            ProfScope ps(c, K_STAMP_SUM, ls);
            launch_stamp_sum(ls, tc, nsum, d_res, res_f32, lsum, nchunk_lane[j] > 0 ? 1 : 0);
        }
        HIPCHK(hipGetLastError());
        if (!dev_out && psf_out) {
            HIPCHK(hipMemcpyAsync(psf_out + (size_t)t0 * nsum * per_stamp, d_res,
                                  (size_t)tc * nsum * per_stamp * sizeof(double),
                                  hipMemcpyDeviceToHost, ls));
        }
        ++nchunk_lane[j];
        c->last_chunk_tasks = tc;
        c->last_lane = (L0 + j) % NLmax;
    }
    hipStream_t s = c->stream;
    for (int j = 0; j < NL; ++j) {
        mpsfr_ctx::Lane& ln = lane_of(j);
        if (zero) {
            ln.marked = false;
        } else if (lean) {
            HIPCHK(hipEventRecord(sl.call_done, ln.stream));
            ln.done_ev = sl.call_done;
            ln.marked = true;
        } else {
            HIPCHK(hipEventRecord(ln.done, ln.stream));
            ln.done_ev = ln.done;
            ln.marked = true;
            HIPCHK(hipStreamWaitEvent(s, ln.done, 0));
        }
        ln.busy = true;
        for (int a = 0; a < 3; ++a) ln.outs[ln.nouts % mpsfr_ctx::Lane::NHIST][a] = outs[a];
        ln.nouts += 1;
// ... 714 lines not shown
```

### muse_psfr_amd/csrc/stage_a2.hip

```cpp
#include <cstdlib>
#include <type_traits>
#include <utility>

#include "device_common.h"
#include "conv_frames.h"
#include "mf_common.h"
#include "dpp_groups.h"
#include "psd_model.h"

namespace mpsfr {

namespace {

constexpr double kEps0 = 1.0 / 128.0;

template <int Q> struct WQ;
template <> struct WQ<8> {
    static constexpr double c[4] = {1.0, 0.70710678118654752440, 0.0, -0.70710678118654752440};
    static constexpr double s[4] = {0.0, -0.70710678118654752440, -1.0, -0.70710678118654752440};
};
template <> struct WQ<16> {
    static constexpr double c[10] = {1.0, 0.92387953251128675613, 0.70710678118654752440, 0.38268343236508977173,
                                     0.0, -0.38268343236508977173, -0.70710678118654752440,
                                     -0.92387953251128675613, -1.0, -0.92387953251128675613};
    static constexpr double s[10] = {0.0, -0.38268343236508977173, -0.70710678118654752440,
                                     -0.92387953251128675613, -1.0, -0.92387953251128675613,
                                     -0.70710678118654752440, -0.38268343236508977173, 0.0,
                                     0.38268343236508977173};
};
template <> struct WQ<20> {
    static constexpr double c[13] = {1.0, 0.95105651629515357212, 0.80901699437494742410,
                                     0.58778525229247312917, 0.30901699437494742410, 0.0,
                                     -0.30901699437494742410, -0.58778525229247312917,
                                     -0.80901699437494742410, -0.95105651629515357212, -1.0,
                                     -0.95105651629515357212, -0.80901699437494742410};
    static constexpr double s[13] = {0.0, -0.30901699437494742410, -0.58778525229247312917,
                                     -0.80901699437494742410, -0.95105651629515357212, -1.0,
                                     -0.95105651629515357212, -0.80901699437494742410,
                                     -0.58778525229247312917, -0.30901699437494742410, 0.0,
                                     0.30901699437494742410, 0.58778525229247312917};
};
template <> struct WQ<4> {
    static constexpr double c[1] = {1.0};
    static constexpr double s[1] = {0.0};
};

template <int M>
__device__ __forceinline__ void dftm(cx<double>* v) {
    if constexpr (M == 2) dft2(v[0], v[1]);
    if constexpr (M == 4) dft4(v[0], v[1], v[2], v[3]);
    if constexpr (M == 5) dft5(v);
}

template <int Q> constexpr int fold_jmin() { return -((NAO / 2 + Q - 1) / Q); }
template <int Q> constexpr int fold_jmax() { return (NAO / 2 + Q - 1) / Q; }
template <int Q> constexpr int fold_nj() { return fold_jmax<Q>() - fold_jmin<Q>(); }
constexpr bool fold_valid(int Q, int r, int j) { return r + Q * j >= -NAO / 2 && r + Q * j < NAO / 2; }

template <int B, int E, typename F>
__device__ __forceinline__ void static_for(F&& f) {
    if constexpr (B < E) {
        f(std::integral_constant<int, B>{});
        static_for<B + 1, E>(f);
    }
}

template <int Q, typename F>
__device__ __forceinline__ void dftq_real_out(F&& G, double* out) {
    static_assert(Q % 4 == 0, "Q = 2 is handled by the caller");
    constexpr int M = Q / 4;
    double t0[M], t1[M], t2[M], t3[M];
    {
        cx<double> v[M];
        G(std::integral_constant<int, 0>{}, v);
        dftm<M>(v);
#pragma unroll
        for (int b = 0; b < M; ++b) t0[b] = v[b].x;
    }
    {
        cx<double> v[M];
        G(std::integral_constant<int, 2>{}, v);
        dftm<M>(v);
#pragma unroll
        for (int b = 0; b < M; ++b) {
            const double re = b == 0 ? v[b].x : v[b].x * WQ<Q>::c[2 * b] - v[b].y * WQ<Q>::s[2 * b];
            t1[b] = t0[b] - re;
            t0[b] = t0[b] + re;
        }
    }
    {
        cx<double> v[M];
        G(std::integral_constant<int, 1>{}, v);
        dftm<M>(v);
#pragma unroll
        for (int b = 0; b < M; ++b) {
            if (b == 0) {
                t2[b] = v[b].x;
                t3[b] = v[b].y;
            } else {
                t2[b] = v[b].x * WQ<Q>::c[b] - v[b].y * WQ<Q>::s[b];
                t3[b] = v[b].x * WQ<Q>::s[b] + v[b].y * WQ<Q>::c[b];
            }
        }
    }
    {
        cx<double> v[M];
        G(std::integral_constant<int, 3>{}, v);
        dftm<M>(v);
#pragma unroll
        for (int b = 0; b < M; ++b) {
            if (b == 0) {
                t2[b] += v[b].x;
                t3[b] -= v[b].y;
            } else {
                t2[b] += v[b].x * WQ<Q>::c[3 * b] - v[b].y * WQ<Q>::s[3 * b];
                t3[b] -= v[b].x * WQ<Q>::s[3 * b] + v[b].y * WQ<Q>::c[3 * b];
            }
        }
    }
#pragma unroll
    for (int b = 0; b < M; ++b) {
        out[b] = t0[b] + t2[b];
        out[2 * M + b] = t0[b] - t2[b];
        out[M + b] = t1[b] + t3[b];
        out[3 * M + b] = t1[b] - t3[b];
    }
}

__device__ __forceinline__ void dft16(cx<double>* v) {
#pragma unroll
    for (int n2 = 0; n2 < 4; ++n2) dft4(v[n2], v[4 + n2], v[8 + n2], v[12 + n2]);
#pragma unroll
    for (int k1 = 1; k1 < 4; ++k1)
#pragma unroll
        for (int n2 = 1; n2 < 4; ++n2) {
            const cx<double> w = {WQ<16>::c[n2 * k1], WQ<16>::s[n2 * k1]};
            v[4 * k1 + n2] = cmul(v[4 * k1 + n2], w);
        }
#pragma unroll
    for (int k1 = 0; k1 < 4; ++k1) dft4(v[4 * k1], v[4 * k1 + 1], v[4 * k1 + 2], v[4 * k1 + 3]);
    cx<double> o[16];
#pragma unroll
    for (int k1 = 0; k1 < 4; ++k1)
#pragma unroll
        for (int k2 = 0; k2 < 4; ++k2) o[k1 + 4 * k2] = v[4 * k1 + k2];
#pragma unroll
    for (int i = 0; i < 16; ++i) v[i] = o[i];
}

template <int Q>
__device__ __forceinline__ void dftq(cx<double>* v) {
    if constexpr (Q == 16) dft16(v);
    else dftr<double, Q>(v);
}

template <int LANE>
__device__ __forceinline__ double mov_bc(double x) {
    double d;
    asm("v_mov_b64_dpp %0, %1 row_newbcast:%2 row_mask:0xf bank_mask:0xf" : "=v"(d) : "v"(x), "n"(LANE));
    return d;
}

constexpr int kNX = NAO / 16;

#define MPSFR_MIN4(ctrl)                                                        \
    "v_min_f32_dpp %0, %0, %0 " ctrl " row_mask:0xf bank_mask:0xf bound_ctrl:1\n\t" \
    "v_min_f32_dpp %1, %1, %1 " ctrl " row_mask:0xf bank_mask:0xf bound_ctrl:1\n\t" \
    "v_min_f32_dpp %2, %2, %2 " ctrl " row_mask:0xf bank_mask:0xf bound_ctrl:1\n\t" \
    "v_min_f32_dpp %3, %3, %3 " ctrl " row_mask:0xf bank_mask:0xf bound_ctrl:1\n\t"
__device__ __forceinline__ void min32_x4(float& a, float& b, float& c, float& d) {
    asm("s_nop 1\n\t"
        MPSFR_MIN4("quad_perm:[1,0,3,2]")
        MPSFR_MIN4("quad_perm:[2,3,0,1]")
        MPSFR_MIN4("row_half_mirror")
        MPSFR_MIN4("row_mirror")
        MPSFR_MIN4("row_bcast:15")
        "s_nop 0"
        : "+v"(a), "+v"(b), "+v"(c), "+v"(d));
}
__device__ __forceinline__ void min16_x4(float& a, float& b, float& c, float& d) {
    asm("s_nop 1\n\t"
        MPSFR_MIN4("quad_perm:[1,0,3,2]")
        MPSFR_MIN4("quad_perm:[2,3,0,1]")
        MPSFR_MIN4("row_half_mirror")
        MPSFR_MIN4("row_mirror")
        "s_nop 0"
        : "+v"(a), "+v"(b), "+v"(c), "+v"(d));
}
#undef MPSFR_MIN4

template <int Q, int R0, int RS, int CNT, int J>
struct FoldValid {
    int n = 0, idx[CNT > 0 ? CNT : 1] = {};
    constexpr FoldValid() {
        for (int i = 0; i < CNT; ++i)
            if (fold_valid(Q, R0 + RS * i, J)) idx[n++] = i;
    }
};

template <int Q, bool CPLX, int R0, int RS, int CNT, int J = fold_jmin<Q>()>
__device__ __forceinline__ void fold_group(cx<double>* acc, const double* xr, const double* xi,
                                           const cx<double>* wj) {
    if constexpr (J < fold_jmax<Q>()) {
        constexpr FoldValid<Q, R0, RS, CNT, J> V;
#define MPSFR_FN(k) (R0 + RS * V.idx[k] + Q * J + NAO / 2)
#define MPSFR_FA(k) acc[V.idx[k]]
#define MPSFR_FX(k) xr[MPSFR_FN(k) / 16], xi[MPSFR_FN(k) / 16]
#define MPSFR_FR(k) xr[MPSFR_FN(k) / 16]
#define MPSFR_FL(k) MPSFR_FN(k) % 16
        if constexpr (J == 0) {
            static_for<0, V.n>([&](auto kc) {
                constexpr int k = decltype(kc)::value;
                acc[V.idx[k]].x += mov_bc<MPSFR_FL(k)>(xr[MPSFR_FN(k) / 16]);
                if constexpr (CPLX) acc[V.idx[k]].y += mov_bc<MPSFR_FL(k)>(xi[MPSFR_FN(k) / 16]);
            });
        } else {
            const cx<double> w = wj[J - fold_jmin<Q>()];
            constexpr int n = V.n;
            static_assert(n <= 5, "group sizes up to 5");
            if constexpr (CPLX) {
                if constexpr (n == 5)
                    cmac_group5<MPSFR_FL(0), MPSFR_FL(1), MPSFR_FL(2), MPSFR_FL(3), MPSFR_FL(4)>(
                        MPSFR_FA(0), MPSFR_FA(1), MPSFR_FA(2), MPSFR_FA(3), MPSFR_FA(4), MPSFR_FX(0), MPSFR_FX(1),
                        MPSFR_FX(2), MPSFR_FX(3), MPSFR_FX(4), w);
                if constexpr (n == 4)
                    cmac_group4<MPSFR_FL(0), MPSFR_FL(1), MPSFR_FL(2), MPSFR_FL(3)>(
                        MPSFR_FA(0), MPSFR_FA(1), MPSFR_FA(2), MPSFR_FA(3), MPSFR_FX(0), MPSFR_FX(1), MPSFR_FX(2),
                        MPSFR_FX(3), w);
                if constexpr (n == 2 || n == 3)
                    cmac_group2<MPSFR_FL(0), MPSFR_FL(1)>(MPSFR_FA(0), MPSFR_FA(1), MPSFR_FX(0), MPSFR_FX(1), w);
                if constexpr (n == 3) cmac_group1<MPSFR_FL(2)>(MPSFR_FA(2), MPSFR_FX(2), w);
                if constexpr (n == 1) cmac_group1<MPSFR_FL(0)>(MPSFR_FA(0), MPSFR_FX(0), w);
            } else {
                if constexpr (n == 5)
                    rmac_group5<MPSFR_FL(0), MPSFR_FL(1), MPSFR_FL(2), MPSFR_FL(3), MPSFR_FL(4)>(
                        MPSFR_FA(0), MPSFR_FA(1), MPSFR_FA(2), MPSFR_FA(3), MPSFR_FA(4), MPSFR_FR(0), MPSFR_FR(1),
                        MPSFR_FR(2), MPSFR_FR(3), MPSFR_FR(4), w);
                if constexpr (n == 4)
                    rmac_group4<MPSFR_FL(0), MPSFR_FL(1), MPSFR_FL(2), MPSFR_FL(3)>(
                        MPSFR_FA(0), MPSFR_FA(1), MPSFR_FA(2), MPSFR_FA(3), MPSFR_FR(0), MPSFR_FR(1), MPSFR_FR(2),
                        MPSFR_FR(3), w);
                if constexpr (n == 2 || n == 3)
                    rmac_group2<MPSFR_FL(0), MPSFR_FL(1)>(MPSFR_FA(0), MPSFR_FA(1), MPSFR_FR(0), MPSFR_FR(1), w);
                if constexpr (n == 3) rmac_group1<MPSFR_FL(2)>(MPSFR_FA(2), MPSFR_FR(2), w);
                if constexpr (n == 1) rmac_group1<MPSFR_FL(0)>(MPSFR_FA(0), MPSFR_FR(0), w);
            }
        }
#undef MPSFR_FN
#undef MPSFR_FA
#undef MPSFR_FX
#undef MPSFR_FR
#undef MPSFR_FL
        fold_group<Q, CPLX, R0, RS, CNT, J + 1>(acc, xr, xi, wj);
    }
}

template <int Q> constexpr int group_cnt() { return Q >= 16 ? Q / 4 : (Q < 4 ? Q : 4); }

template <int Q, bool CPLX, int R0, int RS, int CNT, typename WR>
__device__ __forceinline__ void fold_sums(cx<double>* v, const double* xr, const double* xi,
                                          const cx<double>* wj, WR&& wrf) {
#pragma unroll
    for (int i = 0; i < CNT; ++i) v[i] = {0.0, 0.0};
    fold_group<Q, CPLX, R0, RS, CNT>(v, xr, xi, wj);
#pragma unroll
    for (int i = 0; i < CNT; ++i)
        if (R0 + RS * i > 0) v[i] = cmul(v[i], wrf(R0 + RS * i));
}

template <int N, int L>
__global__ void __launch_bounds__(64) k_series_twiddles(const cx<double>* __restrict__ twg,
                                                        cx<double>* __restrict__ twk) {
    constexpr int Q = N / L, NJ = fold_nj<Q>(), JMIN = fold_jmin<Q>();
    const int row = blockIdx.x, k2 = threadIdx.x;
    if (k2 >= L) return;
    if (row < NJ) twk[row * L + k2] = twg[(((Q * (row + JMIN) * k2) % N) + N) % N];
    else twk[row * L + k2] = twg[((row - NJ) * k2) % N];
}

template <int N>
constexpr int series_lanes() { return N <= 256 ? 16 : (N == 512 ? 32 : 64); }
template <int N, int L>
constexpr size_t twiddle_entries() { return (size_t)(fold_nj<N / L>() + N / L) * L; }

struct ParamCopy {
    uint4* dst;
    const uint4* src;
    int n16;
};
struct ParamFlag {
    unsigned long long* flag;
    unsigned long long seq;
    int* queue_zero;
};

template <bool F64, typename... Mix>
__global__ void __launch_bounds__(256) k_patch_gen(int ndir, const TaskPar* __restrict__ tp,
                                                   const double* __restrict__ aotab, double cfit,
                                                   double* __restrict__ P, ParamCopy pc, Mix... mix) {
    constexpr int NEWTON = F64 ? 2 : 1;
    constexpr int TPW = sizeof(TaskPar) / 8;
    static_assert(sizeof(TaskPar) % 8 == 0, "TaskPar is read in 8-byte words");
    __shared__ unsigned long long tps[TPW];
    const int task = blockIdx.y;
    TaskPar p;
    if (pc.n16 > 0) {
        if (blockIdx.y == gridDim.y - 1) {
            constexpr int PER = 4;
            for (int base = blockIdx.x * 256 * PER; base < pc.n16; base += gridDim.x * 256 * PER) {
                uint4 v[PER];
#pragma unroll
                for (int q = 0; q < PER; ++q) {
                    const int i = base + q * 256 + (int)threadIdx.x;
                    if (i < pc.n16) v[q] = pc.src[i];
                }
#pragma unroll
                for (int q = 0; q < PER; ++q) {
                    const int i = base + q * 256 + (int)threadIdx.x;
                    if (i < pc.n16) pc.dst[i] = v[q];
                }
            }
            return;
        }
        if (threadIdx.x < TPW)
            tps[threadIdx.x] = __builtin_nontemporal_load(reinterpret_cast<const unsigned long long*>(tp + task) + threadIdx.x);
        __syncthreads();
        p = *reinterpret_cast<const TaskPar*>(tps);
    } else {
        p = tp[task];
    }
    const int pix = blockIdx.x * 256 + threadIdx.x;
    if (pix >= NAO * NAO) return;
    const int su = pix / NAO - NAO / 2, sv = pix % NAO - NAO / 2;
    const double fit = psd_fit_value<NEWTON>(su, sv, p, cfit);
    const int ia = su < 0 ? su + NAO : su, ib = sv < 0 ? sv + NAO : sv;
    const double g2 = (double)(su * su + sv * sv) * (1.0 / 256.0);
    const double vk = 0.0229 * p.r0m53 * pow_m11_6<NEWTON>(g2 + p.inv_l0sq);
    const int o = ia * NAO + ib;
    if constexpr (sizeof...(Mix) > 0) {
        const double* w;
        int ntab;
        mix_args(w, ntab, mix...);
        w += (size_t)task * ntab;
        for (int d = 0; d < ndir; ++d) {
            const double* tb = aotab + ((size_t)(p.geom * ndir + d) * (ntab + 1)) * (NAO * NAO);
            double sw = w[0] * tb[o] + w[1] * tb[NAO * NAO + o];
            for (int l = 2; l < ntab; ++l) sw += w[l] * tb[l * NAO * NAO + o];
            const double ao = vk * sw + tb[ntab * NAO * NAO + o];
            P[((size_t)task * ndir + d) * (NAO * NAO) + pix] = fmax(fit, ao) - fit;
        }
        return;
    }
    if (ndir == 1) {
        const double* tb = aotab + ((size_t)p.geom * 3) * (NAO * NAO);
        const double ao = vk * (p.cn2_0 * tb[o] + p.cn2_1 * tb[NAO * NAO + o]) + tb[2 * NAO * NAO + o];
        P[(size_t)task * (NAO * NAO) + pix] = fmax(fit, ao) - fit;
        return;
    }
    for (int d0 = 0; d0 < ndir; d0 += 9) {
        double t0[9], t1[9], t2[9];
#pragma unroll
        for (int i = 0; i < 9; ++i) {
            const int d = min(d0 + i, ndir - 1);
            const double* tb = aotab + ((size_t)(p.geom * ndir + d) * 3) * (NAO * NAO);
            t0[i] = tb[o];
            t1[i] = tb[NAO * NAO + o];
            t2[i] = tb[2 * NAO * NAO + o];
        }
#pragma unroll
        for (int i = 0; i < 9; ++i) {
            if (d0 + i >= ndir) break;
            const double ao = vk * (p.cn2_0 * t0[i] + p.cn2_1 * t1[i]) + t2[i];
            P[((size_t)task * ndir + d0 + i) * (NAO * NAO) + pix] = fmax(fit, ao) - fit;
        }
    }
}

template <int N>
constexpr size_t patch_rows_smem() { return (size_t)(N / 2 + 1) * (4 * (64 / series_lanes<N>()) + 1) * sizeof(cx<double>); }

struct KhatArgs {
    int nker;
    const double* gam;
    const double* alp;
    void* khat;
};

template <int N, typename KR>
constexpr size_t patch_rows_smem_all() {
    if constexpr (std::is_void<KR>::value) return patch_rows_smem<N>();
    else return patch_rows_smem<N>() > conv_smem_bytes<KR>(true) ? patch_rows_smem<N>() : conv_smem_bytes<KR>(true);
}

template <int N, typename KR>
__global__ void __launch_bounds__(256) k_patch_rows(const double* __restrict__ P,
                                                    const cx<double>* __restrict__ twk,
                                                    cx<double>* __restrict__ T, double* __restrict__ sp, int qb,
                                                    int ntd, KhatArgs kh, ParamFlag pf) {
    constexpr int L = series_lanes<N>(), R = 64 / L, Q = N / L, H1 = N / 2 + 1, NJ = fold_nj<Q>();
    if (pf.flag != nullptr && blockIdx.x == 0 && blockIdx.y == 0 && threadIdx.x == 0)
        __hip_atomic_store(pf.flag, pf.seq, __ATOMIC_RELAXED, __HIP_MEMORY_SCOPE_SYSTEM);
    if (pf.queue_zero != nullptr && blockIdx.x == 0 && blockIdx.y == 0 && threadIdx.x == 0) *pf.queue_zero = 0;
    if constexpr (!std::is_void<KR>::value) {
        if ((int)blockIdx.y >= ntd) {
            extern __shared__ __align__(16) unsigned char smem_k[];
            const int kid = ((int)blockIdx.y - ntd) * (int)gridDim.x + (int)blockIdx.x;
            if (kid < kh.nker) khat_body<KR>(kh.gam, kh.alp, (cx<KR>*)kh.khat, smem_k, kid);
            return;
        }
    }
    constexpr bool WJREG = NJ <= 10;
    constexpr int NY = Q / 2 + 1;
    constexpr int RG = 4 * R, RS = RG + 1;
    constexpr int NG = NAO / RG;
    extern __shared__ __align__(16) unsigned char smem[];
    cx<double>* tile = reinterpret_cast<cx<double>*>(smem);
    __shared__ double sred[256];
    const int td = blockIdx.y;
    const double* Pg = P + (size_t)td * (NAO * NAO);
    const int lane = threadIdx.x & 63, rho = lane / L, k2 = lane & (L - 1);
    const int wave = __builtin_amdgcn_readfirstlane(threadIdx.x >> 6);
    const int g_end = min(NG, ((int)blockIdx.x + 1) * qb);
    int g = blockIdx.x * qb;
    double xa[kNX], xb[kNX];
    auto fetch = [&](int gg, double* xr) {
#pragma unroll
        for (int a = 0; a < kNX; ++a) xr[a] = Pg[(RG * gg + R * wave + rho) * NAO + 16 * a + (lane & 15)];
    };
    if (g < g_end) fetch(g, xa);
    if (blockIdx.x == 0) {
        double a = 0.0;
        for (int i = threadIdx.x; i < NAO * NAO; i += 256) a += Pg[i];
        sred[threadIdx.x] = a;
        __syncthreads();
        if (threadIdx.x < 64) {
            double b = (sred[threadIdx.x] + sred[threadIdx.x + 64]) + (sred[threadIdx.x + 128] + sred[threadIdx.x + 192]);
            b = wave_sum(b);
            if (threadIdx.x == 0) sp[td] = b;
        }
    }
    cx<double> wjr[WJREG ? NJ : 1], wr[Q];
    if constexpr (WJREG) {
#pragma unroll
        for (int j = 0; j < NJ; ++j) wjr[j] = twk[j * L + k2];
    }
#pragma unroll
    for (int r = 1; r < Q; ++r) wr[r] = twk[(NJ + r) * L + k2];
    auto pass = [&](int gg, const double* xr) {
        cx<double> S[Q];
        {
            constexpr int GC = Q % 5 == 0 ? 5 : (Q < 4 ? Q : 4);
            cx<double> wl[WJREG ? 1 : NJ];
            if constexpr (!WJREG) {
#pragma unroll
                for (int j = 0; j < NJ; ++j) wl[j] = twk[j * L + k2];
            }
            const cx<double>* wjp = WJREG ? wjr : wl;
            static_for<0, Q / GC>([&](auto gc) {
                constexpr int R0 = decltype(gc)::value * GC;
                fold_sums<Q, false, R0, 1, GC>(S + R0, xr, xr, wjp, [&](int r) { return wr[r]; });
            });
        }
        dftq<Q>(S);
#pragma unroll
        for (int k1 = 0; k1 < NY; ++k1)
            if (L * k1 + k2 <= N / 2) tile[(L * k1 + k2) * RS + R * wave + rho] = S[k1];
        __syncthreads();
        cx<double>* Tt = T + (size_t)td * H1 * NAO + RG * gg;
        for (int e = threadIdx.x; e < H1 * RG; e += 256) {
            const int y = e / RG, i = e % RG;
            Tt[(size_t)y * NAO + i] = tile[y * RS + i];
        }
        __syncthreads();
    };
    while (g < g_end) {
        if (g + 1 < g_end) fetch(g + 1, xb);
        pass(g, xa);
        g += 1;
        if (g >= g_end) break;
        if (g + 1 < g_end) fetch(g + 1, xa);
        pass(g, xb);
        g += 1;
    }
}

template <typename RO> struct SeriesCfg;
template <> struct SeriesCfg<float> { static constexpr int K = 4; };
template <> struct SeriesCfg<double> { static constexpr int K = 8; };

template <int N, typename RO, int L>
__device__ __forceinline__ void series_line(const cx<double>* xv, const cx<double>* wjp,
                                            const cx<double>* swr, const RO* scoef, double r0m53,
                                            double delta, double spv, double scale2, RO* dst, float* dlin,
                                            bool valid, int lane, unsigned kmask) {
    constexpr int Q = N / L, K = SeriesCfg<RO>::K;
    constexpr float kSkipped = 3.0e38f;
    const int k2 = lane & (L - 1);
    double xr[kNX], xi[kNX];
#pragma unroll
    for (int a = 0; a < kNX; ++a) {
        xr[a] = xv[a].x;
        xi[a] = xv[a].y;
    }
    double out[Q];
    int always;
    asm volatile("s_mov_b32 %0, 1" : "=s"(always));
    if (!always) {
#pragma unroll
        for (int k1 = 0; k1 < Q; ++k1) out[k1] = xr[k1 % kNX];
    } else {
        auto wrf = [&](int r) { return swr[r * L + k2]; };
        if constexpr (Q == 2) {
            cx<double> S[2];
            fold_sums<Q, true, 0, 1, 2>(S, xr, xi, wjp, wrf);
            out[0] = S[0].x + S[1].x;
            out[1] = S[0].x - S[1].x;
        } else if constexpr (Q >= 16) {
            dftq_real_out<Q>(
                [&](auto r1c, cx<double>* v) {
                    fold_sums<Q, true, decltype(r1c)::value, 4, Q / 4>(v, xr, xi, wjp, wrf);
                },
                out);
        } else {
            cx<double> S[Q];
            static_for<0, Q / 4>([&](auto gc) {
                constexpr int R0 = decltype(gc)::value * 4;
                fold_sums<Q, true, R0, 1, 4>(S + R0, xr, xi, wjp, wrf);
            });
            dftq_real_out<Q>(
                [&](auto r1c, cx<double>* v) {
#pragma unroll
                    for (int r2 = 0; r2 < Q / 4; ++r2) v[r2] = S[4 * r2 + decltype(r1c)::value];
                },
                out);
        }
    }
    constexpr int NB = L == 16 ? Q / 2 : Q;
    float keep[(NB + 15) / 16], dq[Q < 4 ? 4 : Q];
#pragma unroll
    for (int i = 0; i < (NB + 15) / 16; ++i) keep[i] = 0.f;
    if constexpr (sizeof(RO) == 4) {
        const float df = (float)delta, rf = (float)r0m53;
#pragma unroll
        for (int k1 = 0; k1 < Q; ++k1) {
            if (!((kmask >> k1) & 1u)) {
                dq[k1] = kSkipped;
                continue;
            }
            const float4 h = *reinterpret_cast<const float4*>(scoef + (size_t)(L * k1 + k2) * K);
            const float dF = rf * fmaf(fmaf(fmaf(h.w, df, h.z), df, h.y), df, h.x);
            const float d = (float)(fma(scale2, spv - out[k1], (double)dF));
            if (valid) dst[L * k1] = d;
            dq[k1] = fmaxf(d, 0.f);
        }
    } else {
#pragma unroll
        for (int k1 = 0; k1 < Q; ++k1) {
            if (!((kmask >> k1) & 1u)) {
                dq[k1] = kSkipped;
                continue;
            }
            const double* h = scoef + (size_t)(L * k1 + k2) * K;
            double a = h[K - 1];
#pragma unroll
            for (int k = K - 2; k >= 0; --k) a = fma(a, delta, h[k]);
            const double d = fma(scale2, spv - out[k1], r0m53 * a);
            if (valid) dst[L * k1] = d;
            dq[k1] = fmaxf(__double2float_rd(d), 0.f);
        }
    }
    if (dlin != nullptr) {
        if constexpr (Q < 4) {
            dq[2] = dq[0];
            dq[3] = dq[1];
        }
        if constexpr (L == 16) {
            static_assert(Q % 8 == 0, "pairs of values, four pairs to a statement");
#pragma unroll
            for (int kb = 0; kb < NB; ++kb) dq[kb] = fminf(dq[2 * kb], dq[2 * kb + 1]);
#pragma unroll
            for (int kb = 0; kb < NB; kb += 4) {
                min16_x4(dq[kb], dq[kb + 1], dq[kb + 2], dq[kb + 3]);
#pragma unroll
                for (int i = 0; i < 4; ++i)
                    if ((lane & 15) == ((kb + i) & 15)) keep[(kb + i) >> 4] = dq[kb + i];
            }
            if (valid) {
#pragma unroll
                for (int i = 0; i < (NB + 15) / 16; ++i) {
                    const int kb = 16 * i + (lane & 15);
                    if (kb < NB) dlin[kb] = keep[i];
                }
            }
        } else {
#pragma unroll
            for (int k1 = 0; k1 < (Q < 4 ? 4 : Q); k1 += 4) {
                min32_x4(dq[k1], dq[k1 + 1], dq[k1 + 2], dq[k1 + 3]);
#pragma unroll
                for (int i = 0; i < 4; ++i)
                    if (k1 + i < Q && (lane & 15) == ((k1 + i) & 15)) keep[(k1 + i) >> 4] = dq[k1 + i];
            }
            if (valid && (lane & 16)) {
#pragma unroll
                for (int i = 0; i < (Q + 15) / 16; ++i) {
                    const int k1 = 16 * i + (lane & 15);
                    if (k1 < Q) dlin[L == 64 ? 2 * k1 + (lane >> 5) : k1] = keep[i];
                }
            }
        }
    }
}

#ifndef MPSFR_SERIES_THREADS
#define MPSFR_SERIES_THREADS 512
#endif
template <int N, typename RO>
constexpr int series_threads() { return N <= 128 ? 256 : MPSFR_SERIES_THREADS; }
template <int N, typename RO>
constexpr size_t series_smem() {
    return 2 * (size_t)N * SeriesCfg<RO>::K * sizeof(RO) + (size_t)N * sizeof(cx<double>);
}
template <int N, typename RO>
constexpr bool series_fits() { return series_smem<N, RO>() <= 160 * 1024; }

template <int N, typename RO>
__global__ void __launch_bounds__((series_threads<N, RO>()), (512 / series_threads<N, RO>() > 1 ? 2 : 1))
k_dphi_series(const cx<double>* __restrict__ T, const double* __restrict__ sp,
              const TaskPar* __restrict__ tp, int ndir, int ntd, const RO* __restrict__ coef,
              const cx<double>* __restrict__ twk, double scale2, RO* __restrict__ D0t,
              float* __restrict__ dlin, int* __restrict__ zero17, const unsigned* __restrict__ support) {
    constexpr int L = series_lanes<N>(), R = 64 / L, Q = N / L, H1 = N / 2 + 1, K = SeriesCfg<RO>::K;
    constexpr int THREADS = series_threads<N, RO>(), NW = THREADS / 64, NJ = fold_nj<Q>();
    constexpr bool WJREG = NJ <= 10;
    constexpr int LINE = N * K;
    extern __shared__ __align__(16) unsigned char smem[];
    RO* scoef = reinterpret_cast<RO*>(smem);
    cx<double>* swr = reinterpret_cast<cx<double>*>(smem + 2 * (size_t)LINE * sizeof(RO));
    const int lane = threadIdx.x & 63, rho = lane / L, k2 = lane & (L - 1);
    const int wave = __builtin_amdgcn_readfirstlane(threadIdx.x >> 6);
    const int nq = (ntd + R - 1) / R;
    const long C = (long)H1 * nq;
    const int c0 = (int)(C * blockIdx.x / gridDim.x), c1 = (int)(C * (blockIdx.x + 1) / gridDim.x);
    if (zero17 != nullptr && blockIdx.x == 0 && threadIdx.x < kMfSchedInts) zero17[threadIdx.x] = 0;
    if (c0 >= c1) return;
    cx<double> xva[kNX], xvb[kNX];
    auto fetch = [&](int c, cx<double>* xv) {
        const int y = c / nq, td = min(R * (c - y * nq) + rho, ntd - 1);
        const cx<double>* src = T + ((size_t)td * H1 + y) * NAO + (lane & 15);
#pragma unroll
        for (int a = 0; a < kNX; ++a) xv[a] = src[16 * a];
    };
    const int nwe = min(NW, nq);
    const bool active = wave < nwe;
    if (active && c0 + wave < c1) fetch(c0 + wave, xva);
    using V4 = typename std::conditional<sizeof(RO) == 4, float4, double2>::type;
    constexpr int NV = (int)((size_t)LINE * sizeof(RO) / 16);
    auto load_line = [&](int y) {
        if (y > N / 2) return;
        const V4* src = reinterpret_cast<const V4*>(coef + (size_t)y * LINE);
        V4* dst = reinterpret_cast<V4*>(scoef + (size_t)(y & 1) * LINE);
        for (int i = threadIdx.x; i < NV; i += THREADS) dst[i] = src[i];
    };
    int ylo = c0 / nq;
    load_line(ylo);
    load_line(ylo + 1);
    for (int i = threadIdx.x; i < Q * L; i += THREADS) swr[i] = twk[NJ * L + i];
    cx<double> wjr[WJREG ? NJ : 1];
    if constexpr (WJREG) {
#pragma unroll
        for (int j = 0; j < NJ; ++j) wjr[j] = twk[j * L + k2];
    }
    __syncthreads();
    auto unit = [&](int c, const cx<double>* xv) {
        const int y = c / nq, tdr = R * (c - y * nq) + rho;
        const bool valid = tdr < ntd;
        const int td = valid ? tdr : ntd - 1;
        const int task = td / ndir;
        const double r0m53 = tp[task].r0m53, delta = tp[task].inv_l0sq - kEps0;
        const double spv = sp[td];
        cx<double> wl[WJREG ? 1 : NJ];
        if constexpr (!WJREG) {
#pragma unroll
            for (int j = 0; j < NJ; ++j) wl[j] = twk[j * L + k2];
        }
        const unsigned kmask = support != nullptr ? (unsigned)__builtin_amdgcn_readfirstlane((int)support[y]) : 0xffffffffu;
        series_line<N, RO, L>(xv, WJREG ? wjr : wl, swr, scoef + (size_t)(y & 1) * LINE, r0m53, delta, spv, scale2,
                              D0t + ((size_t)td * H1 + y) * N + k2,
                              dlin != nullptr ? dlin + ((size_t)td * H1 + y) * (N / 32) : nullptr, valid, lane, kmask);
    };
    auto new_y = [&](int cb) {
        const int yb = cb / nq;
        if (yb != ylo) {
            __syncthreads();
            for (int yy = ylo + 2; yy <= yb + 1; ++yy) load_line(yy);
            ylo = yb;
            __syncthreads();
        }
    };
    for (int cb = c0; cb < c1; cb += 2 * nwe) {
        new_y(cb);
        {
            const int c = cb + wave;
            if (active && c + nwe < c1) fetch(c + nwe, xvb);
            if (active && c < c1) unit(c, xva);
        }
        if (cb + nwe < c1) {
            new_y(cb + nwe);
            const int c = cb + nwe + wave;
            if (active && c + nwe < c1) fetch(c + nwe, xva);
            if (active && c < c1) unit(c, xvb);
        }
    }
}

struct SeriesSkip {
    const float* tlmax;
    float c2max;
    float thr_elem;
    float thr_mass;
};

template <int N, typename RO>
constexpr size_t series_q_smem() {
    return 4 * (size_t)N * SeriesCfg<RO>::K * sizeof(RO) + (size_t)N * sizeof(cx<double>);
}
template <int N, typename RO>
constexpr bool series_q_fits() { return series_q_smem<N, RO>() <= 160 * 1024; }

template <int N, typename RO>
__global__ void __launch_bounds__((series_threads<N, RO>()), (512 / series_threads<N, RO>() > 1 ? 2 : 1))
k_dphi_series_q(const cx<double>* __restrict__ T, const double* __restrict__ sp,
                const TaskPar* __restrict__ tp, int ndir, int ntd, const RO* __restrict__ coef,
                const cx<double>* __restrict__ twk, double scale2, RO* __restrict__ D0t,
                float* __restrict__ dlin, int* __restrict__ zero17, const unsigned* __restrict__ support,
                const int* __restrict__ perm, int* __restrict__ queue, SeriesSkip skip) {
    constexpr int L = series_lanes<N>(), R = 64 / L, Q = N / L, H1 = N / 2 + 1, K = SeriesCfg<RO>::K;
    constexpr int THREADS = series_threads<N, RO>(), NW = THREADS / 64, NJ = fold_nj<Q>();
    constexpr bool WJREG = NJ <= 10;
    constexpr int LINE = N * K;
    constexpr int LINE_BYTES = LINE * (int)sizeof(RO), CHUNKS = LINE_BYTES / 1024;
    static_assert(LINE_BYTES % 1024 == 0, "a line is whole 1 KB pieces of LDS-DMA");
    constexpr int GB = NW;
    extern __shared__ __align__(16) unsigned char smem[];
    RO* scoef = reinterpret_cast<RO*>(smem);
    cx<double>* swr = reinterpret_cast<cx<double>*>(smem + 4 * (size_t)LINE * sizeof(RO));
    __shared__ int s_next[2];
    const unsigned lds0 = (unsigned)(size_t)(__attribute__((address_space(3))) unsigned char*)smem;
    const int lane = threadIdx.x & 63, rho = lane / L, k2 = lane & (L - 1);
    const int wave = __builtin_amdgcn_readfirstlane(threadIdx.x >> 6);
    const int nq = (ntd + R - 1) / R;
    const int C = H1 * nq, nblk = (C + GB - 1) / GB;
    if (zero17 != nullptr && blockIdx.x == 0 && threadIdx.x < kMfSchedInts) zero17[threadIdx.x] = 0;
    int blk = blockIdx.x;
    if (blk >= nblk) return;
    auto issue_lines = [&](int b, int set) {
        const int y0 = (b * GB) / nq, y1 = min(C - 1, b * GB + GB - 1) / nq;
        for (int ln = 0; ln <= y1 - y0; ++ln) {
            const char* src = reinterpret_cast<const char*>(coef + (size_t)(y0 + ln) * LINE);
#pragma unroll
            for (int c0 = 0; c0 < CHUNKS; c0 += NW) {
                const int c = c0 + wave;
                if (c < CHUNKS)
                    glds16s(src + (size_t)c * 1024, (unsigned)lane * 16,
                            lds0 + (unsigned)(2 * set + ln) * LINE_BYTES + (unsigned)c * 1024);
            }
        }
    };
    auto unit_of = [&](int b, int u, int& y) -> int {
        const int c = b * GB + u;
        if (c >= C) return -1;
        y = c / nq;
        const int r = R * (c - y * nq) + rho;
        return r < ntd ? (perm != nullptr ? perm[r] : r) : -2;
    };
    const int td_last = perm != nullptr ? perm[ntd - 1] : ntd - 1;
    cx<double> xva[kNX], xvb[kNX];
    auto fetch = [&](int b, int u, cx<double>* xv) {
        int y = 0;
        const int t = unit_of(b, u, y);
        if (t == -1) return;
        const cx<double>* src = T + ((size_t)(t >= 0 ? t : td_last) * H1 + y) * NAO + (lane & 15);
#pragma unroll
        for (int a = 0; a < kNX; ++a) xv[a] = src[16 * a];
    };
    issue_lines(blk, 0);
    fetch(blk, wave, xva);
    for (int i = threadIdx.x; i < Q * L; i += THREADS) swr[i] = twk[NJ * L + i];
    cx<double> wjr[WJREG ? NJ : 1];
    if constexpr (WJREG) {
#pragma unroll
        for (int j = 0; j < NJ; ++j) wjr[j] = twk[j * L + k2];
    }
    if (threadIdx.x == 0) s_next[0] = (int)gridDim.x + atomicAdd(queue, 1);
    asm volatile("s_waitcnt vmcnt(0)" ::: "memory");
    __syncthreads();
    auto unit = [&](int b, int u, const cx<double>* xv, int set) {
        int y = 0;
        const int t = unit_of(b, u, y);
        if (t == -1) return;
        const bool valid = t >= 0;
        const int td = valid ? t : td_last;
        const int task = td / ndir;
        const double r0m53 = tp[task].r0m53, delta = tp[task].inv_l0sq - kEps0;
        const double spv = sp[td];
        cx<double> wl[WJREG ? 1 : NJ];
        if constexpr (!WJREG) {
#pragma unroll
            for (int j = 0; j < NJ; ++j) wl[j] = twk[j * L + k2];
        }
        const unsigned kmask = support != nullptr ? (unsigned)__builtin_amdgcn_readfirstlane((int)support[y]) : 0xffffffffu;
        if (skip.tlmax != nullptr && y >= 4) {
            float m = 0.f;
#pragma unroll
            for (int a = 0; a < kNX; ++a) {
                const float re = (float)xv[a].x, im = (float)xv[a].y;
                m += __builtin_sqrtf(fmaf(re, re, im * im));
            }
#pragma unroll
            for (int o = 1; o < 16; o <<= 1) m += __shfl_xor(m, o, 64);
            const float lb = fmaxf((float)(scale2 * (spv - (double)m * 1.00001)), 0.f);
            const float e = fmaf(skip.c2max, lb, skip.tlmax[y]);
            const bool drop = e < skip.thr_elem || e + (float)(1 + __builtin_ctz(N & -N) + (N == 1280 ? 3 : 0)) < skip.thr_mass;
            if (__all(drop || !valid)) {
                if (valid) {
                    RO* dst = D0t + ((size_t)td * H1 + y) * N + k2;
#pragma unroll
                    for (int k1 = 0; k1 < Q; ++k1)
                        if ((kmask >> k1) & 1u) dst[L * k1] = (RO)1.0e30f;
                    if (dlin != nullptr && k2 < N / 32) dlin[((size_t)td * H1 + y) * (N / 32) + k2] = lb;
                }
                return;
            }
        }
        const int ln = y - (b * GB) / nq;
        series_line<N, RO, L>(xv, WJREG ? wjr : wl, swr, scoef + (size_t)(2 * set + ln) * LINE, r0m53, delta, spv, scale2,
                              D0t + ((size_t)td * H1 + y) * N + k2,
                              dlin != nullptr ? dlin + ((size_t)td * H1 + y) * (N / 32) : nullptr, valid, lane, kmask);
    };
    while (true) {
        int nxt = s_next[0];
        bool more = nxt < nblk;
        if (more) {
            issue_lines(nxt, 1);
            fetch(nxt, wave, xvb);
        }
        unit(blk, wave, xva, 0);
        if (more && threadIdx.x == 0) s_next[1] = (int)gridDim.x + atomicAdd(queue, 1);
        asm volatile("s_waitcnt vmcnt(0)" ::: "memory");
        __syncthreads();
        if (!more) break;
        blk = nxt;
        nxt = s_next[1];
        more = nxt < nblk;
        if (more) {
            issue_lines(nxt, 0);
            fetch(nxt, wave, xva);
        }
        unit(blk, wave, xvb, 1);
        if (more && threadIdx.x == 0) s_next[0] = (int)gridDim.x + atomicAdd(queue, 1);
        asm volatile("s_waitcnt vmcnt(0)" ::: "memory");
        __syncthreads();
        if (!more) break;
        blk = nxt;
    }
}

template <int N, typename RO>
constexpr size_t series1_smem() {
    return (size_t)N * SeriesCfg<RO>::K * sizeof(RO) + (size_t)(N / 64) * 64 * sizeof(cx<double>);
}

template <int N, typename RO>
__global__ void __launch_bounds__(256)
k_dphi_series1(const cx<double>* __restrict__ T, const double* __restrict__ sp,
               const TaskPar* __restrict__ tp, int ndir, int ntd, int tg, const RO* __restrict__ coef,
               const cx<double>* __restrict__ twk, double scale2, RO* __restrict__ D0t,
               float* __restrict__ dlin, int* __restrict__ zero17, const unsigned* __restrict__ support) {
    constexpr int Q = N / 64, H1 = N / 2 + 1, K = SeriesCfg<RO>::K, THREADS = 256;
    constexpr int NJ = fold_nj<Q>(), JMIN = fold_jmin<Q>();
    constexpr bool WJREG = NJ <= 10;
    extern __shared__ __align__(16) unsigned char smem[];
    RO* scoef = reinterpret_cast<RO*>(smem);
    cx<double>* swr = reinterpret_cast<cx<double>*>(smem + (size_t)N * K * sizeof(RO));
    const int y = blockIdx.x, g = blockIdx.y;
    const int lane = threadIdx.x & 63;
    const int wave = __builtin_amdgcn_readfirstlane(threadIdx.x >> 6);
    const int td_end = min(ntd, (g + 1) * tg);
    int td = g * tg + wave;
    cx<double> xva[kNX], xvb[kNX];
    auto fetch = [&](int t, cx<double>* xv) {
        const cx<double>* src = T + ((size_t)t * H1 + y) * NAO + (lane & 15);
#pragma unroll
        for (int a = 0; a < kNX; ++a) xv[a] = src[16 * a];
    };
    if (td < td_end) fetch(td, xva);
    {
        using V4 = typename std::conditional<sizeof(RO) == 4, float4, double2>::type;
        constexpr int NV = (int)((size_t)N * K * sizeof(RO) / 16);
        const V4* src = reinterpret_cast<const V4*>(coef + (size_t)y * N * K);
        V4* dst = reinterpret_cast<V4*>(scoef);
        for (int i = threadIdx.x; i < NV; i += THREADS) dst[i] = src[i];
        for (int i = threadIdx.x; i < Q * 64; i += THREADS) swr[i] = twk[NJ * 64 + i];
    }
    if (zero17 != nullptr && y == 0 && g == 0 && threadIdx.x < kMfSchedInts) zero17[threadIdx.x] = 0;
    cx<double> wjr[WJREG ? NJ : 1];
    if constexpr (WJREG) {
#pragma unroll
        for (int j = 0; j < NJ; ++j) wjr[j] = twk[j * 64 + lane];
    }
    __syncthreads();
    const unsigned kmask = support != nullptr ? (unsigned)__builtin_amdgcn_readfirstlane((int)support[y]) : 0xffffffffu;
    auto line = [&](int td, const cx<double>* xv) {
        const int task = td / ndir;
        const double r0m53 = tp[task].r0m53, delta = tp[task].inv_l0sq - kEps0;
        const double spv = sp[td];
        cx<double> wl[WJREG ? 1 : NJ];
        if constexpr (!WJREG) {
#pragma unroll
            for (int j = 0; j < NJ; ++j) wl[j] = twk[j * 64 + lane];
        }
        series_line<N, RO, 64>(xv, WJREG ? wjr : wl, swr, scoef, r0m53, delta, spv, scale2,
                               D0t + ((size_t)td * H1 + y) * N + lane,
                               dlin != nullptr ? dlin + ((size_t)td * H1 + y) * (N / 32) : nullptr, true, lane, kmask);
    };
    constexpr int STEP = THREADS / 64;
    while (td < td_end) {
        if (td + STEP < td_end) fetch(td + STEP, xvb);
        line(td, xva);
        td += STEP;
        if (td >= td_end) break;
        if (td + STEP < td_end) fetch(td + STEP, xva);
        line(td, xvb);
        td += STEP;
    }
}

template <int N, typename RT>
__global__ void __launch_bounds__(64) k_series_support(const RT* __restrict__ tel, unsigned* __restrict__ support) {
    constexpr int L = series_lanes<N>(), Q = N / L;
    const int y = blockIdx.x, lane = threadIdx.x;
    unsigned m = 0;
    for (int k1 = 0; k1 < Q; ++k1) {
        bool any = false;
        for (int x = L * k1 + lane; x < L * k1 + L; x += 64) any = any || tel[(size_t)y * N + x] > (RT)0;
        if (__ballot(any) != 0ull) m |= 1u << k1;
    }
    if (lane == 0) support[y] = m;
}

template <typename RO>
__global__ void __launch_bounds__(256) k_series_coef(int n, int K, const double* __restrict__ planes,
                                                     RO* __restrict__ coef) {
    const int i = blockIdx.x * 256 + threadIdx.x;
    if (i >= n) return;
    for (int k = 0; k < K; ++k) coef[(size_t)i * K + k] = (RO)planes[(size_t)k * n + i];
}

__global__ void __launch_bounds__(128) k_dmin16(int H1, int nks, const float* __restrict__ dlin,
                                                float* __restrict__ dline, float* __restrict__ dblk) {
    const int mt = blockIdx.x, td = blockIdx.y, nmt = gridDim.x;
    const int nline = min(16, H1 - 16 * mt);
    const float* src = dlin + ((size_t)td * H1 + 16 * mt) * nks;
    if ((int)threadIdx.x < nks) {
        float m = __builtin_inff();
        for (int i = 0; i < nline; ++i) m = fminf(m, src[i * nks + threadIdx.x]);
        dblk[((size_t)td * nmt + mt) * nks + threadIdx.x] = m;
    } else if ((int)threadIdx.x >= 64 && (int)threadIdx.x < 64 + nline) {
        const int i = threadIdx.x - 64;
        float m = __builtin_inff();
        for (int kb = 0; kb < nks; ++kb) m = fminf(m, src[i * nks + kb]);
        dline[(size_t)td * H1 + 16 * mt + i] = m;
    }
}

}

void launch_dmin16(hipStream_t s, int N, int ntd, const float* d_dlin, float* d_dline, float* d_dblk) {
    const int H1 = N / 2 + 1;
    hipLaunchKernelGGL(k_dmin16, dim3((H1 + 15) / 16, ntd), dim3(128), 0, s, H1, N / 32, d_dlin, d_dline, d_dblk);
}

size_t series_twiddle_bytes(int N) {
    size_t n = 0;
    DISPATCH_N(N, { n = (twiddle_entries<NN, 64>() + twiddle_entries<NN, series_lanes<NN>()>()) * sizeof(cx<double>); })
    return n;
}

void launch_series_twiddles(hipStream_t s, int N, const void* d_tw64, void* d_twk) {
    DISPATCH_N(N, {
        constexpr int L = series_lanes<NN>();
        hipLaunchKernelGGL((k_series_twiddles<NN, 64>), dim3(fold_nj<NN / 64>() + NN / 64), dim3(64), 0, s,
                           (const cx<double>*)d_tw64, (cx<double>*)d_twk);
        hipLaunchKernelGGL((k_series_twiddles<NN, L>), dim3(fold_nj<NN / L>() + NN / L), dim3(64), 0, s,
                           (const cx<double>*)d_tw64, (cx<double>*)d_twk + twiddle_entries<NN, 64>());
    })
}

int series_terms(bool f64) { return f64 ? SeriesCfg<double>::K : SeriesCfg<float>::K; }
double series_eps0() { return kEps0; }

void launch_series_support(hipStream_t s, int N, const void* d_tel, bool f64, unsigned* d_support) {
    DISPATCH_N(N, {
        if (f64)
            hipLaunchKernelGGL((k_series_support<NN, double>), dim3(NN / 2 + 1), dim3(64), 0, s, (const double*)d_tel, d_support);
        else
            hipLaunchKernelGGL((k_series_support<NN, float>), dim3(NN / 2 + 1), dim3(64), 0, s, (const float*)d_tel, d_support);
    })
}

void launch_series_coef(hipStream_t s, int N, const double* d_planes, void* d_coef, bool f64) {
    const int n = (N / 2 + 1) * N;
    if (f64)
        hipLaunchKernelGGL(k_series_coef<double>, dim3((n + 255) / 256), dim3(256), 0, s, n,
                           SeriesCfg<double>::K, d_planes, (double*)d_coef);
    else
        hipLaunchKernelGGL(k_series_coef<float>, dim3((n + 255) / 256), dim3(256), 0, s, n,
                           SeriesCfg<float>::K, d_planes, (float*)d_coef);
}

void launch_patch(hipStream_t s, int N, int ntd, int ndir, const TaskPar* d_tp, const double* d_aotab,
                  double cfit, const void* d_twk, double* d_P, void* d_T, double* d_sp, bool f64,
                  const PatchExtras& x, const LayerMix& mix) {
    const int ntask = ntd / ndir;
    const bool copy = x.blob_src != nullptr;
    const dim3 ggrid((NAO * NAO + 255) / 256, ntask + (copy ? 1 : 0));
    ParamCopy pc;
    pc.dst = (uint4*)x.blob_dst; pc.src = (const uint4*)x.blob_src; pc.n16 = copy ? (int)(x.blob_bytes / 16) : 0;
    if (copy) d_tp = x.tp_host;
    if (mix.w != nullptr) {
        if (f64)
            hipLaunchKernelGGL((k_patch_gen<true, const double*, int>), ggrid, dim3(256), 0, s, ndir, d_tp, d_aotab, cfit, d_P, pc,
                               mix.w, mix.ntab);
        else
            hipLaunchKernelGGL((k_patch_gen<false, const double*, int>), ggrid, dim3(256), 0, s, ndir, d_tp, d_aotab, cfit, d_P, pc,
                               mix.w, mix.ntab);
    } else if (f64)
        hipLaunchKernelGGL(k_patch_gen<true>, ggrid, dim3(256), 0, s, ndir, d_tp, d_aotab, cfit, d_P, pc);
    else
        hipLaunchKernelGGL(k_patch_gen<false>, ggrid, dim3(256), 0, s, ndir, d_tp, d_aotab, cfit, d_P, pc);
    ParamFlag pf;
    pf.flag = copy ? x.flag : nullptr; pf.seq = x.seq; pf.queue_zero = x.queue_zero;
    KhatArgs kh;
    kh.nker = x.khat_n; kh.gam = x.khat_gam; kh.alp = x.khat_alp; kh.khat = x.khat_out;
    DISPATCH_N(N, {
        constexpr int NG = NAO * series_lanes<NN>() / 256;
        int nb = (512 + ntd - 1) / ntd;
        if (nb > NG) nb = NG;
        if (nb < 1) nb = 1;
        const int qb = (NG + nb - 1) / nb;
        nb = (NG + qb - 1) / qb;
        const int ky = kh.nker > 0 ? (kh.nker + nb - 1) / nb : 0;
        if (kh.nker <= 0) {
            constexpr size_t sm = patch_rows_smem_all<NN, void>();
            allow_smem((k_patch_rows<NN, void>), sm);
            hipLaunchKernelGGL((k_patch_rows<NN, void>), dim3(nb, ntd), dim3(256), sm, s, (const double*)d_P,
                               (const cx<double>*)d_twk + twiddle_entries<NN, 64>(), (cx<double>*)d_T, d_sp, qb, ntd, kh, pf);
        } else if (x.khat_f64) {
            constexpr size_t sm = patch_rows_smem_all<NN, double>();
            allow_smem((k_patch_rows<NN, double>), sm);
            hipLaunchKernelGGL((k_patch_rows<NN, double>), dim3(nb, ntd + ky), dim3(256), sm, s, (const double*)d_P,
                               (const cx<double>*)d_twk + twiddle_entries<NN, 64>(), (cx<double>*)d_T, d_sp, qb, ntd, kh, pf);
        } else {
            constexpr size_t sm = patch_rows_smem_all<NN, float>();
            allow_smem((k_patch_rows<NN, float>), sm);
            hipLaunchKernelGGL((k_patch_rows<NN, float>), dim3(nb, ntd + ky), dim3(256), sm, s, (const double*)d_P,
                               (const cx<double>*)d_twk + twiddle_entries<NN, 64>(), (cx<double>*)d_T, d_sp, qb, ntd, kh, pf);
        }
    })
}

template <int N, typename RO>
bool series_q_usable(int ntd) {
    constexpr int R = 64 / series_lanes<N>(), GB = series_threads<N, RO>() / 64;
    return series_q_fits<N, RO>() && (ntd + R - 1) / R >= GB;
}

void launch_dphi_series(hipStream_t s, int N, int ntd, int ndir, const TaskPar* d_tp, const void* d_T,
                        const double* d_sp, const void* d_coef, const void* d_twk, double scale2,
                        void* d_D0t, float* d_dlin, bool f64out, int* d_zero, int ncu, const unsigned* d_support,
                        const SeriesQueue& qx) {
    const int H1 = N / 2 + 1;
    SeriesSkip sk;
    sk.tlmax = qx.tlmax; sk.c2max = qx.c2max; sk.thr_elem = qx.thr_elem; sk.thr_mass = qx.thr_mass;
    auto first_form = [&](auto kernel, size_t sm) {
        const int waves = 4;
        int ngr = (2048 + H1 - 1) / H1;
        if (ngr * waves > ntd) ngr = (ntd + waves - 1) / waves;
        if (ngr < 1) ngr = 1;
        int tg = (ntd + ngr - 1) / ngr;
        tg = (tg + waves - 1) / waves * waves;
        ngr = (ntd + tg - 1) / tg;
        return std::make_pair(dim3(H1, ngr), tg);
    };
    DISPATCH_N(N, {
        if (f64out) {
            if constexpr (series_fits<NN, double>()) {
                constexpr size_t sm = series_smem<NN, double>();
                if (qx.queue != nullptr && series_q_usable<NN, double>(ntd)) {
                    constexpr size_t smq = series_q_smem<NN, double>() <= 160 * 1024 ? series_q_smem<NN, double>() : 0;
                    allow_smem((k_dphi_series_q<NN, double>), smq);
                    hipLaunchKernelGGL((k_dphi_series_q<NN, double>), dim3(ncu), dim3(series_threads<NN, double>()), smq, s,
                                       (const cx<double>*)d_T, d_sp, d_tp, ndir, ntd, (const double*)d_coef,
                                       (const cx<double>*)d_twk + twiddle_entries<NN, 64>(), scale2, (double*)d_D0t, d_dlin, d_zero,
                                       d_support, qx.perm, qx.queue, sk);
                    return;
                }
                allow_smem((k_dphi_series<NN, double>), sm);
                hipLaunchKernelGGL((k_dphi_series<NN, double>), dim3(ncu), dim3(series_threads<NN, double>()), sm, s,
                                   (const cx<double>*)d_T, d_sp, d_tp, ndir, ntd, (const double*)d_coef,
                                   (const cx<double>*)d_twk + twiddle_entries<NN, 64>(), scale2, (double*)d_D0t, d_dlin, d_zero, d_support);
            } else {
                constexpr size_t sm = series1_smem<NN, double>();
                allow_smem((k_dphi_series1<NN, double>), sm);
                const auto gt = first_form(0, sm);
                hipLaunchKernelGGL((k_dphi_series1<NN, double>), gt.first, dim3(256), sm, s,
                                   (const cx<double>*)d_T, d_sp, d_tp, ndir, ntd, gt.second, (const double*)d_coef,
                                   (const cx<double>*)d_twk, scale2, (double*)d_D0t, d_dlin, d_zero, d_support);
            }
        } else {
            constexpr size_t sm = series_smem<NN, float>();
            if (qx.queue != nullptr && series_q_usable<NN, float>(ntd)) {
                constexpr size_t smq = series_q_smem<NN, float>();
                allow_smem((k_dphi_series_q<NN, float>), smq);
                hipLaunchKernelGGL((k_dphi_series_q<NN, float>), dim3(ncu), dim3(series_threads<NN, float>()), smq, s,
                                   (const cx<double>*)d_T, d_sp, d_tp, ndir, ntd, (const float*)d_coef,
                                   (const cx<double>*)d_twk + twiddle_entries<NN, 64>(), scale2, (float*)d_D0t, d_dlin, d_zero,
                                   d_support, qx.perm, qx.queue, sk);
                return;
            }
            allow_smem((k_dphi_series<NN, float>), sm);
            hipLaunchKernelGGL((k_dphi_series<NN, float>), dim3(ncu), dim3(series_threads<NN, float>()), sm, s,
                               (const cx<double>*)d_T, d_sp, d_tp, ndir, ntd, (const float*)d_coef,
                               (const cx<double>*)d_twk + twiddle_entries<NN, 64>(), scale2, (float*)d_D0t, d_dlin, d_zero, d_support);
        }
    })
}

}
```

Before: 18.43 million.

## Exploit Hermitian symmetry of intermediate T to halve stored and folded columns

The stage-A2 transform output T now keeps only the non-negative half (NAO/2+1 columns) of a Hermitian-symmetric spectrum instead of all NAO columns. The producer combines conjugate pairs when writing, and the consumers fold the halved input with new conjugate-multiply DPP helpers and a Hermitian real-output DFT. This halves T memory traffic and storage and cuts FMA work in the folding step. The cost is more complex index logic, clamped loads and special handling of the self-conjugate and boundary classes, where a mistake would give wrong results.

Result: faster. 19.09 million, median of 6 (+3.6%).

```diff
diff --git a/muse_psfr_amd/csrc/dpp_groups.h b/muse_psfr_amd/csrc/dpp_groups.h
--- a/muse_psfr_amd/csrc/dpp_groups.h
+++ b/muse_psfr_amd/csrc/dpp_groups.h
@@ -10,6 +10,16 @@
         "v_fmac_f64_dpp %1, %2, %5 row_newbcast:%6 row_mask:0xf bank_mask:0xf\n\t"
         "v_fmac_f64_dpp %0, -%3, %5 row_newbcast:%6 row_mask:0xf bank_mask:0xf\n\t"
         "v_fmac_f64_dpp %1, %3, %4 row_newbcast:%6 row_mask:0xf bank_mask:0xf"
+        : "+v"(a0.x), "+v"(a0.y)
+        : "v"(xr0), "v"(xi0), "v"(w.x), "v"(w.y), "n"(L0));
+}
+
+template <int L0>
+__device__ __forceinline__ void cmacc_group1(cx<double>& a0, double xr0, double xi0, const cx<double>& w) {
+    asm("v_fmac_f64_dpp %0, %2, %4 row_newbcast:%6 row_mask:0xf bank_mask:0xf\n\t"
+        "v_fmac_f64_dpp %1, %2, %5 row_newbcast:%6 row_mask:0xf bank_mask:0xf\n\t"
+        "v_fmac_f64_dpp %0, %3, %5 row_newbcast:%6 row_mask:0xf bank_mask:0xf\n\t"
+        "v_fmac_f64_dpp %1, -%3, %4 row_newbcast:%6 row_mask:0xf bank_mask:0xf"
         : "+v"(a0.x), "+v"(a0.y)
         : "v"(xr0), "v"(xi0), "v"(w.x), "v"(w.y), "n"(L0));
 }
@@ -32,6 +42,20 @@
         "v_fmac_f64_dpp %2, -%7, %9 row_newbcast:%11 row_mask:0xf bank_mask:0xf\n\t"
         "v_fmac_f64_dpp %1, %5, %8 row_newbcast:%10 row_mask:0xf bank_mask:0xf\n\t"
         "v_fmac_f64_dpp %3, %7, %8 row_newbcast:%11 row_mask:0xf bank_mask:0xf"
+        : "+v"(a0.x), "+v"(a0.y), "+v"(a1.x), "+v"(a1.y)
+        : "v"(xr0), "v"(xi0), "v"(xr1), "v"(xi1), "v"(w.x), "v"(w.y), "n"(L0), "n"(L1));
+}
+
+template <int L0, int L1>
+__device__ __forceinline__ void cmacc_group2(cx<double>& a0, cx<double>& a1, double xr0, double xi0, double xr1, double xi1, const cx<double>& w) {
+    asm("v_fmac_f64_dpp %0, %4, %8 row_newbcast:%10 row_mask:0xf bank_mask:0xf\n\t"
+        "v_fmac_f64_dpp %2, %6, %8 row_newbcast:%11 row_mask:0xf bank_mask:0xf\n\t"
+        "v_fmac_f64_dpp %1, %4, %9 row_newbcast:%10 row_mask:0xf bank_mask:0xf\n\t"
+        "v_fmac_f64_dpp %3, %6, %9 row_newbcast:%11 row_mask:0xf bank_mask:0xf\n\t"
+        "v_fmac_f64_dpp %0, %5, %9 row_newbcast:%10 row_mask:0xf bank_mask:0xf\n\t"
+        "v_fmac_f64_dpp %2, %7, %9 row_newbcast:%11 row_mask:0xf bank_mask:0xf\n\t"
+        "v_fmac_f64_dpp %1, -%5, %8 row_newbcast:%10 row_mask:0xf bank_mask:0xf\n\t"
+        "v_fmac_f64_dpp %3, -%7, %8 row_newbcast:%11 row_mask:0xf bank_mask:0xf"
         : "+v"(a0.x), "+v"(a0.y), "+v"(a1.x), "+v"(a1.y)
         : "v"(xr0), "v"(xi0), "v"(xr1), "v"(xi1), "v"(w.x), "v"(w.y), "n"(L0), "n"(L1));
 }
@@ -64,6 +88,28 @@
         "v_fmac_f64_dpp %3, %11, %16 row_newbcast:%19 row_mask:0xf bank_mask:0xf\n\t"
         "v_fmac_f64_dpp %5, %13, %16 row_newbcast:%20 row_mask:0xf bank_mask:0xf\n\t"
         "v_fmac_f64_dpp %7, %15, %16 row_newbcast:%21 row_mask:0xf bank_mask:0xf"
+        : "+v"(a0.x), "+v"(a0.y), "+v"(a1.x), "+v"(a1.y), "+v"(a2.x), "+v"(a2.y), "+v"(a3.x), "+v"(a3.y)
+        : "v"(xr0), "v"(xi0), "v"(xr1), "v"(xi1), "v"(xr2), "v"(xi2), "v"(xr3), "v"(xi3), "v"(w.x), "v"(w.y), "n"(L0), "n"(L1), "n"(L2), "n"(L3));
+}
+
+template <int L0, int L1, int L2, int L3>
+__device__ __forceinline__ void cmacc_group4(cx<double>& a0, cx<double>& a1, cx<double>& a2, cx<double>& a3, double xr0, double xi0, double xr1, double xi1, double xr2, double xi2, double xr3, double xi3, const cx<double>& w) {
+    asm("v_fmac_f64_dpp %0, %8, %16 row_newbcast:%18 row_mask:0xf bank_mask:0xf\n\t"
+        "v_fmac_f64_dpp %2, %10, %16 row_newbcast:%19 row_mask:0xf bank_mask:0xf\n\t"
+        "v_fmac_f64_dpp %4, %12, %16 row_newbcast:%20 row_mask:0xf bank_mask:0xf\n\t"
+        "v_fmac_f64_dpp %6, %14, %16 row_newbcast:%21 row_mask:0xf bank_mask:0xf\n\t"
+        "v_fmac_f64_dpp %1, %8, %17 row_newbcast:%18 row_mask:0xf bank_mask:0xf\n\t"
+        "v_fmac_f64_dpp %3, %10, %17 row_newbcast:%19 row_mask:0xf bank_mask:0xf\n\t"
+        "v_fmac_f64_dpp %5, %12, %17 row_newbcast:%20 row_mask:0xf bank_mask:0xf\n\t"
+        "v_fmac_f64_dpp %7, %14, %17 row_newbcast:%21 row_mask:0xf bank_mask:0xf\n\t"
+        "v_fmac_f64_dpp %0, %9, %17 row_newbcast:%18 row_mask:0xf bank_mask:0xf\n\t"
+        "v_fmac_f64_dpp %2, %11, %17 row_newbcast:%19 row_mask:0xf bank_mask:0xf\n\t"
+        "v_fmac_f64_dpp %4, %13, %17 row_newbcast:%20 row_mask:0xf bank_mask:0xf\n\t"
+        "v_fmac_f64_dpp %6, %15, %17 row_newbcast:%21 row_mask:0xf bank_mask:0xf\n\t"
+        "v_fmac_f64_dpp %1, -%9, %16 row_newbcast:%18 row_mask:0xf bank_mask:0xf\n\t"
+        "v_fmac_f64_dpp %3, -%11, %16 row_newbcast:%19 row_mask:0xf bank_mask:0xf\n\t"
+        "v_fmac_f64_dpp %5, -%13, %16 row_newbcast:%20 row_mask:0xf bank_mask:0xf\n\t"
+        "v_fmac_f64_dpp %7, -%15, %16 row_newbcast:%21 row_mask:0xf bank_mask:0xf"
         : "+v"(a0.x), "+v"(a0.y), "+v"(a1.x), "+v"(a1.y), "+v"(a2.x), "+v"(a2.y), "+v"(a3.x), "+v"(a3.y)
         : "v"(xr0), "v"(xi0), "v"(xr1), "v"(xi1), "v"(xr2), "v"(xi2), "v"(xr3), "v"(xi3), "v"(w.x), "v"(w.y), "n"(L0), "n"(L1), "n"(L2), "n"(L3));
 }
@@ -109,6 +155,32 @@
 }
 
 template <int L0, int L1, int L2, int L3, int L4>
+__device__ __forceinline__ void cmacc_group5(cx<double>& a0, cx<double>& a1, cx<double>& a2, cx<double>& a3, cx<double>& a4, double xr0, double xi0, double xr1, double xi1, double xr2, double xi2, double xr3, double xi3, double xr4, double xi4, const cx<double>& w) {
+    asm("v_fmac_f64_dpp %0, %10, %20 row_newbcast:%22 row_mask:0xf bank_mask:0xf\n\t"
+        "v_fmac_f64_dpp %2, %12, %20 row_newbcast:%23 row_mask:0xf bank_mask:0xf\n\t"
+        "v_fmac_f64_dpp %4, %14, %20 row_newbcast:%24 row_mask:0xf bank_mask:0xf\n\t"
+        "v_fmac_f64_dpp %6, %16, %20 row_newbcast:%25 row_mask:0xf bank_mask:0xf\n\t"
+        "v_fmac_f64_dpp %8, %18, %20 row_newbcast:%26 row_mask:0xf bank_mask:0xf\n\t"
+        "v_fmac_f64_dpp %1, %10, %21 row_newbcast:%22 row_mask:0xf bank_mask:0xf\n\t"
+        "v_fmac_f64_dpp %3, %12, %21 row_newbcast:%23 row_mask:0xf bank_mask:0xf\n\t"
+        "v_fmac_f64_dpp %5, %14, %21 row_newbcast:%24 row_mask:0xf bank_mask:0xf\n\t"
+        "v_fmac_f64_dpp %7, %16, %21 row_newbcast:%25 row_mask:0xf bank_mask:0xf\n\t"
+        "v_fmac_f64_dpp %9, %18, %21 row_newbcast:%26 row_mask:0xf bank_mask:0xf\n\t"
+        "v_fmac_f64_dpp %0, %11, %21 row_newbcast:%22 row_mask:0xf bank_mask:0xf\n\t"
+        "v_fmac_f64_dpp %2, %13, %21 row_newbcast:%23 row_mask:0xf bank_mask:0xf\n\t"
+        "v_fmac_f64_dpp %4, %15, %21 row_newbcast:%24 row_mask:0xf bank_mask:0xf\n\t"
+        "v_fmac_f64_dpp %6, %17, %21 row_newbcast:%25 row_mask:0xf bank_mask:0xf\n\t"
+        "v_fmac_f64_dpp %8, %19, %21 row_newbcast:%26 row_mask:0xf bank_mask:0xf\n\t"
+        "v_fmac_f64_dpp %1, -%11, %20 row_newbcast:%22 row_mask:0xf bank_mask:0xf\n\t"
+        "v_fmac_f64_dpp %3, -%13, %20 row_newbcast:%23 row_mask:0xf bank_mask:0xf\n\t"
+        "v_fmac_f64_dpp %5, -%15, %20 row_newbcast:%24 row_mask:0xf bank_mask:0xf\n\t"
+        "v_fmac_f64_dpp %7, -%17, %20 row_newbcast:%25 row_mask:0xf bank_mask:0xf\n\t"
+        "v_fmac_f64_dpp %9, -%19, %20 row_newbcast:%26 row_mask:0xf bank_mask:0xf"
+        : "+v"(a0.x), "+v"(a0.y), "+v"(a1.x), "+v"(a1.y), "+v"(a2.x), "+v"(a2.y), "+v"(a3.x), "+v"(a3.y), "+v"(a4.x), "+v"(a4.y)
+        : "v"(xr0), "v"(xi0), "v"(xr1), "v"(xi1), "v"(xr2), "v"(xi2), "v"(xr3), "v"(xi3), "v"(xr4), "v"(xi4), "v"(w.x), "v"(w.y), "n"(L0), "n"(L1), "n"(L2), "n"(L3), "n"(L4));
+}
+
+template <int L0, int L1, int L2, int L3, int L4>
 __device__ __forceinline__ void rmac_group5(cx<double>& a0, cx<double>& a1, cx<double>& a2, cx<double>& a3, cx<double>& a4, double xr0, double xr1, double xr2, double xr3, double xr4, const cx<double>& w) {
     asm("v_fmac_f64_dpp %0, %10, %15 row_newbcast:%17 row_mask:0xf bank_mask:0xf\n\t"
         "v_fmac_f64_dpp %2, %11, %15 row_newbcast:%18 row_mask:0xf bank_mask:0xf\n\t"
diff --git a/muse_psfr_amd/csrc/kernels.h b/muse_psfr_amd/csrc/kernels.h
--- a/muse_psfr_amd/csrc/kernels.h
+++ b/muse_psfr_amd/csrc/kernels.h
@@ -8,6 +8,7 @@
 constexpr int NSH = NS / 2 + 1;
 constexpr int KS = 41;
 constexpr int NAO = 80;
+constexpr int kNH = NAO / 2 + 1;
 constexpr int NFIT = 16;
 constexpr int NFIT_ELL = 24;
 constexpr int NFIT_PSF = 16;
diff --git a/muse_psfr_amd/csrc/mpsfr_api.cpp b/muse_psfr_amd/csrc/mpsfr_api.cpp
--- a/muse_psfr_amd/csrc/mpsfr_api.cpp
+++ b/muse_psfr_amd/csrc/mpsfr_api.cpp
@@ -1110,7 +1110,7 @@
         const int soft = (4096 + spt - 1) / spt < 8 ? 8 : (4096 + spt - 1) / spt;
         if (big > 512) big = 512;
         if (big < soft) big = soft;
-        const double per_task = series ? (double)ndir * H1 * (N * (double)rsize(c) + NAO * 16.0)
+        const double per_task = series ? (double)ndir * H1 * (N * (double)rsize(c) + kNH * 16.0)
                                        : (double)ndir * (N / 2 + NAO / 2) * H1 * 16.0;
         const int cap = (int)(4.0 * 1024 * 1024 * 1024 / per_task);
         if (big > cap) big = cap < 1 ? 1 : cap;
@@ -1438,7 +1438,7 @@
         if (io.pre_in) continue;
         if (series) {
             if ((rc = ensure(c, ln.pP, (size_t)TC * ndir * NAO * NAO * sizeof(double)))) return rc;
-            if ((rc = ensure(c, ln.pT, (size_t)TC * ndir * H1 * NAO * 2 * sizeof(double)))) return rc;
+            if ((rc = ensure(c, ln.pT, (size_t)TC * ndir * H1 * kNH * 2 * sizeof(double)))) return rc;
             if ((rc = ensure(c, ln.psp, (size_t)TC * ndir * sizeof(double)))) return rc;
             if (c->stage_a_queue && (rc = ensure(c, ln.squeue, 64))) return rc;
             if (prune && (rc = ensure(c, ln.dlin, (size_t)TC * ndir * H1 * (N / 32) * sizeof(float)))) return rc;
diff --git a/muse_psfr_amd/csrc/stage_a2.hip b/muse_psfr_amd/csrc/stage_a2.hip
--- a/muse_psfr_amd/csrc/stage_a2.hip
+++ b/muse_psfr_amd/csrc/stage_a2.hip
@@ -15,34 +15,41 @@
 constexpr double kEps0 = 1.0 / 128.0;
 
 template <int Q> struct WQ;
+template <> struct WQ<4> {
+    static constexpr double c[4] = {1.0, 0.0, -1.0, 0.0};
+    static constexpr double s[4] = {0.0, -1.0, 0.0, 1.0};
+};
 template <> struct WQ<8> {
-    static constexpr double c[4] = {1.0, 0.70710678118654752440, 0.0, -0.70710678118654752440};
-    static constexpr double s[4] = {0.0, -0.70710678118654752440, -1.0, -0.70710678118654752440};
+    static constexpr double c[8] = {1.0, 0.70710678118654752440, 0.0, -0.70710678118654752440, -1.0,
+                                    -0.70710678118654752440, 0.0, 0.70710678118654752440};
+    static constexpr double s[8] = {0.0, -0.70710678118654752440, -1.0, -0.70710678118654752440, 0.0,
+                                    0.70710678118654752440, 1.0, 0.70710678118654752440};
 };
 template <> struct WQ<16> {
-    static constexpr double c[10] = {1.0, 0.92387953251128675613, 0.70710678118654752440, 0.38268343236508977173,
-                                     0.0, -0.38268343236508977173, -0.70710678118654752440,
-                                     -0.92387953251128675613, -1.0, -0.92387953251128675613};
-    static constexpr double s[10] = {0.0, -0.38268343236508977173, -0.70710678118654752440,
-                                     -0.92387953251128675613, -1.0, -0.92387953251128675613,
-                                     -0.70710678118654752440, -0.38268343236508977173, 0.0,
+    static constexpr double c[16] = {1.0, 0.92387953251128675613, 0.70710678118654752440, 0.38268343236508977173,
+                                     0.0, -0.38268343236508977173, -0.70710678118654752440, -0.92387953251128675613,
+                                     -1.0, -0.92387953251128675613, -0.70710678118654752440,
+                                     -0.38268343236508977173, 0.0, 0.38268343236508977173, 0.70710678118654752440,
+                                     0.92387953251128675613};
+    static constexpr double s[16] = {0.0, -0.38268343236508977173, -0.70710678118654752440, -0.92387953251128675613,
+                                     -1.0, -0.92387953251128675613, -0.70710678118654752440,
+                                     -0.38268343236508977173, 0.0, 0.38268343236508977173, 0.70710678118654752440,
+                                     0.92387953251128675613, 1.0, 0.92387953251128675613, 0.70710678118654752440,
                                      0.38268343236508977173};
 };
 template <> struct WQ<20> {
-    static constexpr double c[13] = {1.0, 0.95105651629515357212, 0.80901699437494742410,
-                                     0.58778525229247312917, 0.30901699437494742410, 0.0,
-                                     -0.30901699437494742410, -0.58778525229247312917,
+    static constexpr double c[20] = {1.0, 0.95105651629515357212, 0.80901699437494742410, 0.58778525229247312917,
+                                     0.30901699437494742410, 0.0, -0.30901699437494742410, -0.58778525229247312917,
                                      -0.80901699437494742410, -0.95105651629515357212, -1.0,
-                                     -0.95105651629515357212, -0.80901699437494742410};
-    static constexpr double s[13] = {0.0, -0.30901699437494742410, -0.58778525229247312917,
-                                     -0.80901699437494742410, -0.95105651629515357212, -1.0,
-                                     -0.95105651629515357212, -0.80901699437494742410,
-                                     -0.58778525229247312917, -0.30901699437494742410, 0.0,
-                                     0.30901699437494742410, 0.58778525229247312917};
-};
-template <> struct WQ<4> {
-    static constexpr double c[1] = {1.0};
-    static constexpr double s[1] = {0.0};
+                                     -0.95105651629515357212, -0.80901699437494742410, -0.58778525229247312917,
+                                     -0.30901699437494742410, 0.0, 0.30901699437494742410, 0.58778525229247312917,
+                                     0.80901699437494742410, 0.95105651629515357212};
+    static constexpr double s[20] = {0.0, -0.30901699437494742410, -0.58778525229247312917, -0.80901699437494742410,
+                                     -0.95105651629515357212, -1.0, -0.95105651629515357212,
+                                     -0.80901699437494742410, -0.58778525229247312917, -0.30901699437494742410, 0.0,
+                                     0.30901699437494742410, 0.58778525229247312917, 0.80901699437494742410,
+                                     0.95105651629515357212, 1.0, 0.95105651629515357212, 0.80901699437494742410,
+                                     0.58778525229247312917, 0.30901699437494742410};
 };
 
 template <int M>
@@ -57,6 +64,11 @@
 template <int Q> constexpr int fold_nj() { return fold_jmax<Q>() - fold_jmin<Q>(); }
 constexpr bool fold_valid(int Q, int r, int j) { return r + Q * j >= -NAO / 2 && r + Q * j < NAO / 2; }
 
+constexpr bool hfold_valid(int Q, int r, int j) {
+    const int su = r + Q * j;
+    return su >= -NAO / 2 && su <= NAO / 2 && (2 * r != Q || j >= 0);
+}
+
 template <int B, int E, typename F>
 __device__ __forceinline__ void static_for(F&& f) {
     if constexpr (B < E) {
@@ -65,32 +77,65 @@
     }
 }
 
-template <int Q, typename F>
-__device__ __forceinline__ void dftq_real_out(F&& G, double* out) {
+template <int Q, int MM>
+__device__ __forceinline__ double re_w(const cx<double>& z) {
+    constexpr int m = ((MM % Q) + Q) % Q;
+    constexpr double c = WQ<Q>::c[m], s = WQ<Q>::s[m];
+    if constexpr (c == 1.0) return z.x;
+    else if constexpr (c == -1.0) return -z.x;
+    else if constexpr (s == 1.0) return -z.y;
+    else if constexpr (s == -1.0) return z.y;
+    else return fma(-s, z.y, c * z.x);
+}
+template <int Q, int MM>
+__device__ __forceinline__ double add_re_w(double acc, const cx<double>& z) {
+    constexpr int m = ((MM % Q) + Q) % Q;
+    constexpr double c = WQ<Q>::c[m], s = WQ<Q>::s[m];
+    if constexpr (c == 1.0) return acc + z.x;
+    else if constexpr (c == -1.0) return acc - z.x;
+    else if constexpr (s == 1.0) return acc - z.y;
+    else if constexpr (s == -1.0) return acc + z.y;
+    else return fma(-s, z.y, fma(c, z.x, acc));
+}
+
+template <int Q, typename FE, typename FO>
+__device__ __forceinline__ void dftq_herm_real_out(double s0, FE&& EV, FO&& OD, double* out) {
     static_assert(Q % 4 == 0, "Q = 2 is handled by the caller");
     constexpr int M = Q / 4;
     double t0[M], t1[M], t2[M], t3[M];
     {
-        cx<double> v[M];
-        G(std::integral_constant<int, 0>{}, v);
-        dftm<M>(v);
-#pragma unroll
-        for (int b = 0; b < M; ++b) t0[b] = v[b].x;
+        cx<double> e[M];
+        EV(e);
+        const double sh = e[M - 1].x;
+        static_for<0, M>([&](auto bc) {
+            constexpr int b = decltype(bc)::value;
+            const double shb = b % 2 ? -sh : sh;
+            double v0, v2;
+            if constexpr (M % 2 == 0) {
+                v0 = s0 + shb;
+                v2 = re_w<Q, 2 * b>(e[0]);
+            } else {
+                v0 = s0;
+                v2 = shb;
+            }
+            static_for<(M % 2 == 0 ? 1 : 0), M - 1>([&](auto ic) {
+                constexpr int r = 2 + 2 * decltype(ic)::value;
+                if constexpr (r % 4 == 0) v0 = add_re_w<Q, r * b>(v0, e[decltype(ic)::value]);
+                else v2 = add_re_w<Q, r * b>(v2, e[decltype(ic)::value]);
+            });
+            t0[b] = v0 + v2;
+            t1[b] = v0 - v2;
+        });
     }
     {
-        cx<double> v[M];
-        G(std::integral_constant<int, 2>{}, v);
-        dftm<M>(v);
-#pragma unroll
-        for (int b = 0; b < M; ++b) {
-            const double re = b == 0 ? v[b].x : v[b].x * WQ<Q>::c[2 * b] - v[b].y * WQ<Q>::s[2 * b];
-            t1[b] = t0[b] - re;
-            t0[b] = t0[b] + re;
-        }
-    }
-    {
-        cx<double> v[M];
-        G(std::integral_constant<int, 1>{}, v);
+        cx<double> o[M], v[M];
+        OD(o);
+#pragma unroll
+        for (int r2 = 0; r2 < M; ++r2) {
+            const int r = 4 * r2 + 1;
+            if (2 * r < Q) v[r2] = o[(r - 1) / 2];
+            else v[r2] = {o[(Q - r - 1) / 2].x, -o[(Q - r - 1) / 2].y};
+        }
         dftm<M>(v);
 #pragma unroll
         for (int b = 0; b < M; ++b) {
@@ -103,21 +148,6 @@
             }
         }
     }
-    {
-        cx<double> v[M];
-        G(std::integral_constant<int, 3>{}, v);
-        dftm<M>(v);
-#pragma unroll
-        for (int b = 0; b < M; ++b) {
-            if (b == 0) {
-                t2[b] += v[b].x;
-                t3[b] -= v[b].y;
-            } else {
-                t2[b] += v[b].x * WQ<Q>::c[3 * b] - v[b].y * WQ<Q>::s[3 * b];
-                t3[b] -= v[b].x * WQ<Q>::s[3 * b] + v[b].y * WQ<Q>::c[3 * b];
-            }
-        }
-    }
 #pragma unroll
     for (int b = 0; b < M; ++b) {
         out[b] = t0[b] + t2[b];
@@ -161,7 +191,13 @@
     return d;
 }
 
+template <int LANE>
+__device__ __forceinline__ void fmac_bc(double& acc, double x, double w) {
+    asm("v_fmac_f64_dpp %0, %1, %2 row_newbcast:%3 row_mask:0xf bank_mask:0xf" : "+v"(acc) : "v"(x), "v"(w), "n"(LANE));
+}
+
 constexpr int kNX = NAO / 16;
+constexpr int kNXH = (kNH + 15) / 16;
 
 #define MPSFR_MIN4(ctrl)                                                        \
     "v_min_f32_dpp %0, %0, %0 " ctrl " row_mask:0xf bank_mask:0xf bound_ctrl:1\n\t" \
@@ -189,83 +225,96 @@
 }
 #undef MPSFR_MIN4
 
-template <int Q, int R0, int RS, int CNT, int J>
+template <int Q, bool HERM, int R0, int RS, int CNT, int J>
 struct FoldValid {
     int n = 0, idx[CNT > 0 ? CNT : 1] = {};
     constexpr FoldValid() {
         for (int i = 0; i < CNT; ++i)
-            if (fold_valid(Q, R0 + RS * i, J)) idx[n++] = i;
+            if (HERM ? hfold_valid(Q, R0 + RS * i, J) : fold_valid(Q, R0 + RS * i, J)) idx[n++] = i;
     }
 };
 
-template <int Q, bool CPLX, int R0, int RS, int CNT, int J = fold_jmin<Q>()>
+template <int Q, bool HERM, int R0, int RS, int CNT, int J = fold_jmin<Q>()>
 __device__ __forceinline__ void fold_group(cx<double>* acc, const double* xr, const double* xi,
                                            const cx<double>* wj) {
     if constexpr (J < fold_jmax<Q>()) {
-        constexpr FoldValid<Q, R0, RS, CNT, J> V;
-#define MPSFR_FN(k) (R0 + RS * V.idx[k] + Q * J + NAO / 2)
+        constexpr FoldValid<Q, HERM, R0, RS, CNT, J> V;
+#define MPSFR_FSU(k) (R0 + RS * V.idx[k] + Q * J)
+#define MPSFR_FN(k) (HERM ? (MPSFR_FSU(k) < 0 ? -MPSFR_FSU(k) : MPSFR_FSU(k)) : MPSFR_FSU(k) + NAO / 2)
 #define MPSFR_FA(k) acc[V.idx[k]]
 #define MPSFR_FX(k) xr[MPSFR_FN(k) / 16], xi[MPSFR_FN(k) / 16]
 #define MPSFR_FR(k) xr[MPSFR_FN(k) / 16]
 #define MPSFR_FL(k) MPSFR_FN(k) % 16
+#define MPSFR_FGROUPS(mac, X)                                                                                  \
+    if constexpr (n == 5)                                                                                      \
+        mac##_group5<MPSFR_FL(0), MPSFR_FL(1), MPSFR_FL(2), MPSFR_FL(3), MPSFR_FL(4)>(                         \
+            MPSFR_FA(0), MPSFR_FA(1), MPSFR_FA(2), MPSFR_FA(3), MPSFR_FA(4), X(0), X(1), X(2), X(3), X(4), w); \
+    if constexpr (n == 4)                                                                                      \
+        mac##_group4<MPSFR_FL(0), MPSFR_FL(1), MPSFR_FL(2), MPSFR_FL(3)>(                                      \
+            MPSFR_FA(0), MPSFR_FA(1), MPSFR_FA(2), MPSFR_FA(3), X(0), X(1), X(2), X(3), w);                    \
+    if constexpr (n == 2 || n == 3)                                                                            \
+        mac##_group2<MPSFR_FL(0), MPSFR_FL(1)>(MPSFR_FA(0), MPSFR_FA(1), X(0), X(1), w);                       \
+    if constexpr (n == 3) mac##_group1<MPSFR_FL(2)>(MPSFR_FA(2), X(2), w);                                     \
+    if constexpr (n == 1) mac##_group1<MPSFR_FL(0)>(MPSFR_FA(0), X(0), w);
         if constexpr (J == 0) {
             static_for<0, V.n>([&](auto kc) {
                 constexpr int k = decltype(kc)::value;
                 acc[V.idx[k]].x += mov_bc<MPSFR_FL(k)>(xr[MPSFR_FN(k) / 16]);
-                if constexpr (CPLX) acc[V.idx[k]].y += mov_bc<MPSFR_FL(k)>(xi[MPSFR_FN(k) / 16]);
+                if constexpr (HERM) acc[V.idx[k]].y += mov_bc<MPSFR_FL(k)>(xi[MPSFR_FN(k) / 16]);
             });
         } else {
             const cx<double> w = wj[J - fold_jmin<Q>()];
             constexpr int n = V.n;
             static_assert(n <= 5, "group sizes up to 5");
-            if constexpr (CPLX) {
-                if constexpr (n == 5)
-                    cmac_group5<MPSFR_FL(0), MPSFR_FL(1), MPSFR_FL(2), MPSFR_FL(3), MPSFR_FL(4)>(
-                        MPSFR_FA(0), MPSFR_FA(1), MPSFR_FA(2), MPSFR_FA(3), MPSFR_FA(4), MPSFR_FX(0), MPSFR_FX(1),
-                        MPSFR_FX(2), MPSFR_FX(3), MPSFR_FX(4), w);
-                if constexpr (n == 4)
-                    cmac_group4<MPSFR_FL(0), MPSFR_FL(1), MPSFR_FL(2), MPSFR_FL(3)>(
-                        MPSFR_FA(0), MPSFR_FA(1), MPSFR_FA(2), MPSFR_FA(3), MPSFR_FX(0), MPSFR_FX(1), MPSFR_FX(2),
-                        MPSFR_FX(3), w);
-                if constexpr (n == 2 || n == 3)
-                    cmac_group2<MPSFR_FL(0), MPSFR_FL(1)>(MPSFR_FA(0), MPSFR_FA(1), MPSFR_FX(0), MPSFR_FX(1), w);
-                if constexpr (n == 3) cmac_group1<MPSFR_FL(2)>(MPSFR_FA(2), MPSFR_FX(2), w);
-                if constexpr (n == 1) cmac_group1<MPSFR_FL(0)>(MPSFR_FA(0), MPSFR_FX(0), w);
+            if constexpr (!HERM) {
+                MPSFR_FGROUPS(rmac, MPSFR_FR)
+            } else if constexpr (J < 0) {
+                MPSFR_FGROUPS(cmacc, MPSFR_FX)
             } else {
-                if constexpr (n == 5)
-                    rmac_group5<MPSFR_FL(0), MPSFR_FL(1), MPSFR_FL(2), MPSFR_FL(3), MPSFR_FL(4)>(
-                        MPSFR_FA(0), MPSFR_FA(1), MPSFR_FA(2), MPSFR_FA(3), MPSFR_FA(4), MPSFR_FR(0), MPSFR_FR(1),
-                        MPSFR_FR(2), MPSFR_FR(3), MPSFR_FR(4), w);
-                if constexpr (n == 4)
-                    rmac_group4<MPSFR_FL(0), MPSFR_FL(1), MPSFR_FL(2), MPSFR_FL(3)>(
-                        MPSFR_FA(0), MPSFR_FA(1), MPSFR_FA(2), MPSFR_FA(3), MPSFR_FR(0), MPSFR_FR(1), MPSFR_FR(2),
-                        MPSFR_FR(3), w);
-                if constexpr (n == 2 || n == 3)
-                    rmac_group2<MPSFR_FL(0), MPSFR_FL(1)>(MPSFR_FA(0), MPSFR_FA(1), MPSFR_FR(0), MPSFR_FR(1), w);
-                if constexpr (n == 3) rmac_group1<MPSFR_FL(2)>(MPSFR_FA(2), MPSFR_FR(2), w);
-                if constexpr (n == 1) rmac_group1<MPSFR_FL(0)>(MPSFR_FA(0), MPSFR_FR(0), w);
-            }
-        }
+                MPSFR_FGROUPS(cmac, MPSFR_FX)
+            }
+        }
+#undef MPSFR_FGROUPS
+#undef MPSFR_FSU
 #undef MPSFR_FN
 #undef MPSFR_FA
 #undef MPSFR_FX
 #undef MPSFR_FR
 #undef MPSFR_FL
-        fold_group<Q, CPLX, R0, RS, CNT, J + 1>(acc, xr, xi, wj);
-    }
-}
-
-template <int Q> constexpr int group_cnt() { return Q >= 16 ? Q / 4 : (Q < 4 ? Q : 4); }
-
-template <int Q, bool CPLX, int R0, int RS, int CNT, typename WR>
+        fold_group<Q, HERM, R0, RS, CNT, J + 1>(acc, xr, xi, wj);
+    }
+}
+
+template <int Q, bool HERM, int R0, int RS, int CNT, typename WR>
 __device__ __forceinline__ void fold_sums(cx<double>* v, const double* xr, const double* xi,
                                           const cx<double>* wj, WR&& wrf) {
 #pragma unroll
     for (int i = 0; i < CNT; ++i) v[i] = {0.0, 0.0};
-    fold_group<Q, CPLX, R0, RS, CNT>(v, xr, xi, wj);
-#pragma unroll
-    for (int i = 0; i < CNT; ++i)
-        if (R0 + RS * i > 0) v[i] = cmul(v[i], wrf(R0 + RS * i));
+    fold_group<Q, HERM, R0, RS, CNT>(v, xr, xi, wj);
+#pragma unroll
+    for (int i = 0; i < CNT; ++i) {
+        const int r = R0 + RS * i;
+        if (HERM && 2 * r == Q) {
+            const cx<double> w = wrf(r);
+            v[i] = {fma(-v[i].y, w.y, v[i].x * w.x), 0.0};
+        } else if (r > 0) {
+            v[i] = cmul(v[i], wrf(r));
+        }
+    }
+}
+
+template <int Q, int J = fold_jmin<Q>()>
+__device__ __forceinline__ void fold_class0(double& a, double& b, const double* xr, const double* xi,
+                                            const cx<double>* wj) {
+    if constexpr (J < 0) {
+        if constexpr (Q * J >= -NAO / 2) {
+            constexpr int n = -Q * J;
+            const cx<double> w = wj[J - fold_jmin<Q>()];
+            fmac_bc<n % 16>(a, xr[n / 16], w.x);
+            fmac_bc<n % 16>(b, xi[n / 16], w.y);
+        }
+        fold_class0<Q, J + 1>(a, b, xr, xi, wj);
+    }
 }
 
 template <int N, int L>
@@ -412,6 +461,7 @@
     constexpr bool WJREG = NJ <= 10;
     constexpr int NY = Q / 2 + 1;
     constexpr int RG = 4 * R, RS = RG + 1;
+    constexpr int RH = RG / 2;
     constexpr int NG = NAO / RG;
     extern __shared__ __align__(16) unsigned char smem[];
     cx<double>* tile = reinterpret_cast<cx<double>*>(smem);
@@ -424,8 +474,10 @@
     int g = blockIdx.x * qb;
     double xa[kNX], xb[kNX];
     auto fetch = [&](int gg, double* xr) {
-#pragma unroll
-        for (int a = 0; a < kNX; ++a) xr[a] = Pg[(RG * gg + R * wave + rho) * NAO + 16 * a + (lane & 15)];
+        const int q = R * wave + rho, i = RH * gg + (q < RH ? q : q - RH);
+        const int row = q < RH ? i : (i == 0 ? NAO / 2 : NAO - i);
+#pragma unroll
+        for (int a = 0; a < kNX; ++a) xr[a] = Pg[row * NAO + 16 * a + (lane & 15)];
     };
     if (g < g_end) fetch(g, xa);
     if (blockIdx.x == 0) {
@@ -466,10 +518,16 @@
         for (int k1 = 0; k1 < NY; ++k1)
             if (L * k1 + k2 <= N / 2) tile[(L * k1 + k2) * RS + R * wave + rho] = S[k1];
         __syncthreads();
-        cx<double>* Tt = T + (size_t)td * H1 * NAO + RG * gg;
-        for (int e = threadIdx.x; e < H1 * RG; e += 256) {
-            const int y = e / RG, i = e % RG;
-            Tt[(size_t)y * NAO + i] = tile[y * RS + i];
+        cx<double>* Tt = T + (size_t)td * H1 * kNH;
+        for (int e = threadIdx.x; e < H1 * RH; e += 256) {
+            const int y = e / RH, sl = e % RH, i = RH * gg + sl;
+            const cx<double> vn = tile[y * RS + sl], vp = tile[y * RS + RH + sl];
+            if (i == 0) {
+                Tt[(size_t)y * kNH + NAO / 2] = {vn.x, -vn.y};
+                Tt[(size_t)y * kNH] = {vp.x, 0.0};
+            } else {
+                Tt[(size_t)y * kNH + NAO / 2 - i] = {vp.x + vn.x, vp.y - vn.y};
+            }
         }
         __syncthreads();
     };
@@ -496,9 +554,9 @@
     constexpr int Q = N / L, K = SeriesCfg<RO>::K;
     constexpr float kSkipped = 3.0e38f;
     const int k2 = lane & (L - 1);
-    double xr[kNX], xi[kNX];
-#pragma unroll
-    for (int a = 0; a < kNX; ++a) {
+    double xr[kNXH], xi[kNXH];
+#pragma unroll
+    for (int a = 0; a < kNXH; ++a) {
         xr[a] = xv[a].x;
         xi[a] = xv[a].y;
     }
@@ -507,32 +565,22 @@
     asm volatile("s_mov_b32 %0, 1" : "=s"(always));
     if (!always) {
 #pragma unroll
-        for (int k1 = 0; k1 < Q; ++k1) out[k1] = xr[k1 % kNX];
+        for (int k1 = 0; k1 < Q; ++k1) out[k1] = xr[k1 % kNXH];
     } else {
         auto wrf = [&](int r) { return swr[r * L + k2]; };
+        static_assert((NAO / 2) % Q == 0 || (NAO / 2) % Q == Q / 2, "su = +-40 falls in a self-conjugate class");
+        double s0 = mov_bc<0>(xr[0]), s0b = 0.0;
+        fold_class0<Q>(s0, s0b, xr, xi, wjp);
+        s0 += s0b;
         if constexpr (Q == 2) {
-            cx<double> S[2];
-            fold_sums<Q, true, 0, 1, 2>(S, xr, xi, wjp, wrf);
-            out[0] = S[0].x + S[1].x;
-            out[1] = S[0].x - S[1].x;
-        } else if constexpr (Q >= 16) {
-            dftq_real_out<Q>(
-                [&](auto r1c, cx<double>* v) {
-                    fold_sums<Q, true, decltype(r1c)::value, 4, Q / 4>(v, xr, xi, wjp, wrf);
-                },
-                out);
+            cx<double> S[1];
+            fold_sums<Q, true, 1, 2, 1>(S, xr, xi, wjp, wrf);
+            out[0] = s0 + S[0].x;
+            out[1] = s0 - S[0].x;
         } else {
-            cx<double> S[Q];
-            static_for<0, Q / 4>([&](auto gc) {
-                constexpr int R0 = decltype(gc)::value * 4;
-                fold_sums<Q, true, R0, 1, 4>(S + R0, xr, xi, wjp, wrf);
-            });
-            dftq_real_out<Q>(
-                [&](auto r1c, cx<double>* v) {
-#pragma unroll
-                    for (int r2 = 0; r2 < Q / 4; ++r2) v[r2] = S[4 * r2 + decltype(r1c)::value];
-                },
-                out);
+            dftq_herm_real_out<Q>(
+                s0, [&](cx<double>* v) { fold_sums<Q, true, 2, 2, Q / 4>(v, xr, xi, wjp, wrf); },
+                [&](cx<double>* v) { fold_sums<Q, true, 1, 2, Q / 4>(v, xr, xi, wjp, wrf); }, out);
         }
     }
     constexpr int NB = L == 16 ? Q / 2 : Q;
@@ -643,12 +691,12 @@
     const int c0 = (int)(C * blockIdx.x / gridDim.x), c1 = (int)(C * (blockIdx.x + 1) / gridDim.x);
     if (zero17 != nullptr && blockIdx.x == 0 && threadIdx.x < kMfSchedInts) zero17[threadIdx.x] = 0;
     if (c0 >= c1) return;
-    cx<double> xva[kNX], xvb[kNX];
+    cx<double> xva[kNXH], xvb[kNXH];
     auto fetch = [&](int c, cx<double>* xv) {
         const int y = c / nq, td = min(R * (c - y * nq) + rho, ntd - 1);
-        const cx<double>* src = T + ((size_t)td * H1 + y) * NAO + (lane & 15);
-#pragma unroll
-        for (int a = 0; a < kNX; ++a) xv[a] = src[16 * a];
+        const cx<double>* src = T + ((size_t)td * H1 + y) * kNH;
+#pragma unroll
+        for (int a = 0; a < kNXH; ++a) xv[a] = src[min(16 * a + (lane & 15), kNH - 1)];
     };
     const int nwe = min(NW, nq);
     const bool active = wave < nwe;
@@ -774,14 +822,14 @@
         return r < ntd ? (perm != nullptr ? perm[r] : r) : -2;
     };
     const int td_last = perm != nullptr ? perm[ntd - 1] : ntd - 1;
-    cx<double> xva[kNX], xvb[kNX];
+    cx<double> xva[kNXH], xvb[kNXH];
     auto fetch = [&](int b, int u, cx<double>* xv) {
         int y = 0;
         const int t = unit_of(b, u, y);
         if (t == -1) return;
-        const cx<double>* src = T + ((size_t)(t >= 0 ? t : td_last) * H1 + y) * NAO + (lane & 15);
-#pragma unroll
-        for (int a = 0; a < kNX; ++a) xv[a] = src[16 * a];
+        const cx<double>* src = T + ((size_t)(t >= 0 ? t : td_last) * H1 + y) * kNH;
+#pragma unroll
+        for (int a = 0; a < kNXH; ++a) xv[a] = src[min(16 * a + (lane & 15), kNH - 1)];
     };
     issue_lines(blk, 0);
     fetch(blk, wave, xva);
@@ -812,9 +860,9 @@
         if (skip.tlmax != nullptr && y >= 4) {
             float m = 0.f;
 #pragma unroll
-            for (int a = 0; a < kNX; ++a) {
+            for (int a = 0; a < kNXH; ++a) {
                 const float re = (float)xv[a].x, im = (float)xv[a].y;
-                m += __builtin_sqrtf(fmaf(re, re, im * im));
+                if (16 * a + (lane & 15) < kNH) m += __builtin_sqrtf(fmaf(re, re, im * im));
             }
 #pragma unroll
             for (int o = 1; o < 16; o <<= 1) m += __shfl_xor(m, o, 64);
@@ -887,11 +935,11 @@
     const int wave = __builtin_amdgcn_readfirstlane(threadIdx.x >> 6);
     const int td_end = min(ntd, (g + 1) * tg);
     int td = g * tg + wave;
-    cx<double> xva[kNX], xvb[kNX];
+    cx<double> xva[kNXH], xvb[kNXH];
     auto fetch = [&](int t, cx<double>* xv) {
-        const cx<double>* src = T + ((size_t)t * H1 + y) * NAO + (lane & 15);
-#pragma unroll
-        for (int a = 0; a < kNX; ++a) xv[a] = src[16 * a];
+        const cx<double>* src = T + ((size_t)t * H1 + y) * kNH;
+#pragma unroll
+        for (int a = 0; a < kNXH; ++a) xv[a] = src[min(16 * a + (lane & 15), kNH - 1)];
     };
     if (td < td_end) fetch(td, xva);
     {
```
